# aelmiger/LINE-MOD-Pipeline

Hardware: AMD Instinct MI355X
Metric: detections/sec (higher is better)
Workload: dtype u8

## Files before the change

line-mod-pipeline_amd/csrc/lm_common.h:

```cpp
#pragma once
#include <stdint.h>

typedef uint8_t u8;
typedef uint16_t u16;
typedef uint32_t u32;
typedef uint64_t u64;

#define LM_SCAN_CHUNK 1008
#define LM_SCAN4_CHUNK 1016
#define LM_SCAN_FPAD 8
#define LM_SCANL_LDS_BYTES 163840
#define LM_SCANL_IMAGE_MAX 153600
#define LM_SCANL_TABLE_BYTES 2048
#define LM_SCANL_POS_BITS 15
#define LM_SORT_CAP 4096
#define LM_SORT_CHUNK 1024
#define LM_INLINE_MATCHES 2048
#define LM_DROPPED 0xFFFFFFFFu

struct LmLevelGeom {
    int w, h;
    int T;
    int W, H;
    int spread_only;
    int nibble;
    u32 wh;
    u32 ori_stride;
    u32 plane_ori;
    u32 mod_stride;
    u32 zero_off;
    u32 arena_bytes;
};

struct LmCand {
    u32 ti;
    int x, y;
    float sim;
};

struct LmRefFeat {
    u32 off;
    int16_t x, y;
};

struct LmRefMeta {
    int width, height;
    int nfeat_total;
    u32 start[2];
    u32 count[2];
};

struct LmDevHeader {
    u32 cand_count;
    u32 match_count;
    u32 pad[2];
};

struct LmOutMatch { int x, y; float similarity; int template_id; int class_idx; };

struct LmHeader {
    u32 cand_count;
    u32 match_count;
    u32 out_count;
    u32 sorted_on_device;
};

struct LmHostBlock {
    LmHeader hdr;
    LmOutMatch rec[LM_INLINE_MATCHES];
};
```

line-mod-pipeline_amd/csrc/lm_detector.hip:

```cpp
#include "lm_detector_impl.h"

namespace lmd {

thread_local std::string g_err;
int fail(int code, const std::string& msg) { g_err = msg; return code; }

bool any_lane_busy(const lm_detector* d) {
    for (const lm_detector::Lane& ln : d->lanes) if (ln.busy) return true;
    return false;
}

void free_device_bank(lm_detector* d) {
    hipFree(d->d_item_t); hipFree(d->d_item_chunk); hipFree(d->d_scan_off); hipFree(d->d_scan_P);
    hipFree(d->d_scan_n); hipFree(d->d_t_global); hipFree(d->d_t_class);
    hipFree(d->d_off1); hipFree(d->d_offn); hipFree(d->d_offs3); d->d_off1 = d->d_offn = d->d_offs3 = nullptr;
    hipFree(d->d_offl); hipFree(d->d_offsl); hipFree(d->d_litem); d->d_offl = d->d_offsl = d->d_litem = nullptr;
    for (auto& it : d->items1) { hipFree(it.d_t); hipFree(it.d_chunk); }
    d->items1.clear();
    d->d_item_t = d->d_item_chunk = d->d_scan_off = nullptr;
    d->d_scan_P = d->d_scan_n = d->d_t_global = d->d_t_class = nullptr;
    for (int l = 0; l < LM_MAX_LEVELS; ++l) {
        hipFree(d->d_ref_meta[l]); hipFree(d->d_ref_feat[l]);
        d->d_ref_meta[l] = nullptr; d->d_ref_feat[l] = nullptr;
    }
// ... 357 lines not shown
            for (int l = 0; l < L; ++l) lmk_color_quantize(ln.stream, d->bgr(first, l), d->lw[l], d->lh[l], c.weak_threshold, d->quant(first, l, 0), nullptr, d->cscratch(first, l), fs, n, true);
        grads_done = true;
    }
    for (int l = 0; l < L; ++l) {
        if (l > 0 && !(l == 1 && blur_pyr)) lmk_pyrdown(ln.stream, d->bgr(first, l - 1), d->lw[l - 1], d->lh[l - 1], d->bgr(first, l), fs, n);
        if (!grads_done)
        lmk_color_quantize(ln.stream, d->bgr(first, l), d->lw[l], d->lh[l], c.weak_threshold, d->quant(first, l, 0),
                           nullptr, d->cscratch(first, l), fs, n, l == 0 && blur_pyr);
        if (M == 2 && l == 0)
            lmk_depth_quantize(ln.stream, d->depth(first), d->lw[0], d->lh[0], c.distance_threshold,
                               c.difference_threshold, d->d_normal_lut, normal_lut_onehot(d), d->quant(first, 0, 1),
                               d->dscratch(first), fs, n);
    }
    if (masked) {
        enqueue_mask_rules(d, ln, first, n);
        enqueue_match_masks(d, ln, first, n);
    }
    if (M == 2 && L > 2) enqueue_depth_pyramid(d, ln, first, n);
    for (int l = 0; l < L; ++l)
        for (int m = 0; m < M; ++m) enqueue_lm(d, ln, first, n, l, m, l == L - 1 ? planes : 0u);
}

void fill_raw_thr(int* tab, float threshold) {
    for (int n = 0; n < 128; ++n) tab[n] = static_cast<int>(2 * n + (threshold / 100.f) * (2 * n) + 0.5f);
}

int item_range(lm_detector* d, int class_idx, ItemRange* r) {
    const int nc = (int)d->bank.classes.size();
    if (class_idx >= nc || class_idx < -1) return fail(LM_ERR_INVALID, "class index out of range");
    if (class_idx < 0) { r->lo = 0; r->n = (int)d->hb.item_t.size(); r->t_lo = 0; r->t_hi = (int)d->hb.t_global.size(); }
    else {
        r->lo = d->hb.class_item_lo[class_idx]; r->n = d->hb.class_item_hi[class_idx] - r->lo;
        r->t_lo = d->hb.class_t_lo[class_idx]; r->t_hi = d->hb.class_t_hi[class_idx];
    }
    return LM_OK;
}

int item_ranges(lm_detector* d, std::vector<int>& classes, std::vector<ItemRange>& out) {
    const int nc = (int)d->bank.classes.size();
    out.clear();
    for (int c : classes) if (c < -1 || c >= nc) return fail(LM_ERR_INVALID, "class index out of range");
    std::sort(classes.begin(), classes.end());
    classes.erase(std::unique(classes.begin(), classes.end()), classes.end());
    if (classes.empty() || classes[0] < 0) {
        if (classes.size() > 1) return fail(LM_ERR_INVALID, "class index -1 (all classes) cannot be combined with others");
        classes.assign(1, -1);
        out.push_back(ItemRange{0, (int)d->hb.item_t.size(), 0, (int)d->hb.t_global.size()});
        return LM_OK;
    }
    for (int c : classes) {
        const int lo = d->hb.class_item_lo[c], hi = d->hb.class_item_hi[c];
        if (!out.empty() && out.back().lo + out.back().n == lo && out.back().t_hi == d->hb.class_t_lo[c]) { out.back().n += hi - lo; out.back().t_hi = d->hb.class_t_hi[c]; }
        else out.push_back(ItemRange{lo, hi - lo, d->hb.class_t_lo[c], d->hb.class_t_hi[c]});
    }
    return LM_OK;
}

int ensure_items1(lm_detector* d, int L1, const lm_detector::Items1** out) {
    for (const auto& it : d->items1) if (it.L == L1) { *out = &it; return LM_OK; }
    std::vector<u32> t, c;
    lm_detector::Items1 it;
    it.L = L1;
    lmh::build_items1(d->hb, L1, t, c, it.begin);
    int rc;
    if ((rc = upload_vec(&it.d_t, t))) return rc;
    if ((rc = upload_vec(&it.d_chunk, c))) { hipFree(it.d_t); return rc; }
    d->items1.push_back(std::move(it));
    *out = &d->items1.back();
    return LM_OK;
}

static unsigned slot_layouts(const lm_detector* d, int first, int n) {
    unsigned held = 0;
    for (int i = first; i < first + n; ++i) held |= lmh::layout_bit(d->slots[i].layout);
    return held;
}

static int refuse_scan(lmh::ScanPlan::Kind k) {
    if (k == lmh::ScanPlan::Mixed)
        return fail(LM_ERR_INVALID, "the slots were prepared by calls of different scan forms (some keep only the spread byte of the scanned level): match them apart or upload again");
    return fail(LM_ERR_HIP, "the slots keep only the spread byte of the scanned level and the bit-plane scan could not be set up for them: upload the frames again");
}

int make_scan_args(lm_detector* d, lm_detector::Lane& ln, int first, ItemRange r, int nslots, LmScanArgs* out) {
    const int L = d->cfg.pyramid_levels;
    const LmLevelGeom& g = d->geom[L - 1];
    const unsigned held = slot_layouts(d, first, nslots);
    const bool spread = held == lmh::layout_bit(lmh::Layout::SpreadAndPlanes);
    const int lo = d->hb.lds_ok ? d->hb.lbegin[(size_t)r.t_lo] : 0, nl = d->hb.lds_ok ? d->hb.lbegin[(size_t)r.t_hi] - lo : 0;
    lmh::ScanPlan p = lmh::plan_scan(scan_inputs(d, ln), nslots, held, nl);
    const lm_detector::Items1* it = nullptr;
    if (p.kind == lmh::ScanPlan::Scan1 && ensure_items1(d, p.param, &it) != LM_OK)
        p.kind = spread ? lmh::ScanPlan::NoBitPlaneForm : lmh::ScanPlan::Scan4;
    if (p.kind == lmh::ScanPlan::Mixed || p.kind == lmh::ScanPlan::NoBitPlaneForm) return refuse_scan(p.kind);
    LmScanArgs& a = *out;
    a.L1 = 0; a.G1 = 1; a.L1_rcp16 = 0; a.delta_rcp16 = 0; a.off1 = a.offn = nullptr; a.fpad1 = 0; a.no_exact = 0; a.surv = nullptr; a.surv_cap = 0; a.surv_set = 0; a.exact_spread = 0; a.offs3 = nullptr; a.resp_tab = nullptr;
    a.lm = d->lm(first, L - 1); a.lm_slot_stride = d->frame_stride;
    a.item_t = d->d_item_t; a.item_chunk = d->d_item_chunk;
    a.item_lo = r.lo; a.n_items = r.n;
    a.scan_off = d->d_scan_off; a.scan_P = d->d_scan_P; a.scan_n = d->d_scan_n;
    a.M = d->cfg.num_modalities; a.fpad = d->hb.fpad; a.nibble = g.nibble;
    a.raw_thr_by_n = ln.d_raw_thr;
    a.stat = d->scan_stats ? d->d_scan_stat : nullptr;
    a.W = g.W; a.T = g.T;
    a.hdr = reinterpret_cast<LmDevHeader*>(d->aux(first, d->off_hdr));
    a.cand = reinterpret_cast<LmCand*>(d->aux(first, d->off_cand));
    a.aux_slot_stride = d->aux_stride;
    a.cand_cap = d->max_cand;
    a.dbg = 0; a.lds_form = 0; a.R = 1; a.offl = a.offsl = a.litem = nullptr; a.litem_lo = a.n_litems = 0; a.pb = a.mod_stride = a.planes_off = a.plane_ori = a.tbl_bytes = a.queue_cap = 0;
    if (p.kind != lmh::ScanPlan::Scan4) {
        a.delta_rcp16 = (65536u + (u32)d->miss_delta - 1u) / (u32)d->miss_delta;
        a.fpad1 = d->hb.fpad1; a.exact_spread = spread ? 1 : 0; a.offs3 = d->d_offs3; a.resp_tab = d->d_resp_tab;
    }
    if (p.kind == lmh::ScanPlan::ScanL) {
        a.lds_form = 1; a.R = p.param;
        a.offl = d->d_offl; a.offsl = d->d_offsl; a.litem = d->d_litem; a.litem_lo = lo; a.n_litems = nl;
        a.pb = (u32)g.T * (u32)g.T * g.wh / 8u; a.mod_stride = g.mod_stride; a.planes_off = 8u * g.ori_stride; a.plane_ori = g.plane_ori;
        const u32 img = (u32)a.M * 8u * a.pb;
        a.tbl_bytes = std::max<u32>(LM_SCANL_TABLE_BYTES, (((g.wh + 127u) / 128u) * 16u + 32u + 15u) & ~15u);
        a.queue_cap = std::min<u32>((LM_SCANL_LDS_BYTES - img - a.tbl_bytes - 16u - 512u) / 4u, 1u << 16);
    } else if (p.kind == lmh::ScanPlan::Scan1) {
        const int L1 = p.param;
        a.L1 = L1; a.G1 = 64 / L1;
        a.L1_rcp16 = (65536u + (u32)L1 - 1u) / (u32)L1;
        a.off1 = d->d_off1; a.offn = d->d_offn;
        a.item_t = it->d_t; a.item_chunk = it->d_chunk;
        a.item_lo = it->begin[(size_t)r.t_lo]; a.n_items = it->begin[(size_t)r.t_hi] - a.item_lo;
        unsigned long long*& q = ln.d_surv;
        if (!q) {
            if (hipMalloc(reinterpret_cast<void**>(&q), (16 + (size_t)d->surv_cap) * sizeof(unsigned long long)) != hipSuccess) { q = nullptr; (void)hipGetLastError(); }
            else if (hipMemsetAsync(q, 0, 16 * sizeof(unsigned long long), ln.stream) != hipSuccess) { hipFree(q); q = nullptr; (void)hipGetLastError(); }
            ln.surv_set = 0;
        }
        a.surv = q; a.surv_cap = d->surv_cap;
        a.surv_set = ln.surv_set;
        if (g.wh >= (1u << 20) || nslots > 4096) a.surv = nullptr;
    }
    return LM_OK;
}

void launch_scan(lm_detector::Lane& ln, LmScanArgs& a, int variant, int nslots) {
    lmk_scan(ln.stream, a, variant, nslots);
    if (!a.L1 || !a.surv) return;
    ln.surv_set ^= 1;
    a.surv_set = ln.surv_set;
}

LmRefineArgs make_refine_args(lm_detector* d, int first, int level, float threshold) {
    LmRefineArgs a;
    a.lm = d->lm(first, level); a.lm_slot_stride = d->frame_stride;
    a.g = d->geom[level];
    a.M = d->cfg.num_modalities;
    a.meta = d->d_ref_meta[level]; a.feats = d->d_ref_feat[level];
    a.sim_lut = d->d_sim_lut;
    a.hdr = reinterpret_cast<LmDevHeader*>(d->aux(first, d->off_hdr));
    a.cand = reinterpret_cast<LmCand*>(d->aux(first, d->off_cand));
    a.keys = reinterpret_cast<u64*>(d->aux(first, d->off_keys));
    a.aux_slot_stride = d->aux_stride;
    a.cand_cap = d->max_cand; a.match_cap = d->max_match;
    a.threshold = threshold;
    a.t_global = d->d_t_global; a.t_class = d->d_t_class;
    a.plan = nullptr; a.plan_cap = 0;
    a.stat = d->d_refine_stat;
    return a;
}

LmSortArgs make_sort_args(lm_detector* d, int first) {
    LmSortArgs a;
    a.hdr = reinterpret_cast<LmDevHeader*>(d->aux(first, d->off_hdr));
    a.keys = reinterpret_cast<u64*>(d->aux(first, d->off_keys));
    a.out = reinterpret_cast<LmOutMatch*>(d->aux(first, d->off_out));
    a.split = d->sort_split_mode == 1 || (d->sort_split_mode == 2 && d->sort_long_score > 0);
    a.aux_slot_stride = d->aux_stride;
    a.host = d->host_block(first);
    a.host_slot_stride = d->host_stride;
    a.cand_cap = d->max_cand; a.match_cap = d->max_match;
    return a;
}

int enqueue_threshold(lm_detector::Lane& ln, float threshold) {
    if (!(threshold >= 0.0f)) return fail(LM_ERR_INVALID, "threshold must be >= 0");
    if (ln.raw_thr_for != threshold) {
        HIP_TRY(hipStreamSynchronize(ln.stream));
        fill_raw_thr(ln.h_raw_thr, threshold);
        HIP_TRY(hipMemcpyAsync(ln.d_raw_thr, ln.h_raw_thr, 128 * sizeof(int), hipMemcpyHostToDevice, ln.stream));
        ln.raw_thr_for = threshold;
    }
    return LM_OK;
}

int enqueue_match_stages(lm_detector* d, lm_detector::Lane& ln, int first, int n, float threshold, const std::vector<ItemRange>& ranges, bool timed) {
    const int L = d->cfg.pyramid_levels;
    if (lmh::layouts_mixed(slot_layouts(d, first, n))) return refuse_scan(lmh::ScanPlan::Mixed);
    if (timed) HIP_TRY(hipEventRecord(ln.ev[1], ln.stream));
    for (const ItemRange& r : ranges)
        if (r.n > 0) {
            LmScanArgs sa;
            if (int rc = make_scan_args(d, ln, first, r, n, &sa)) return rc;
            launch_scan(ln, sa, d->scan_variant, n);
            d->cnt_scan_launches += 1; d->cnt_scan1_launches += (sa.L1 || sa.lds_form) ? 1 : 0; d->last_scan1_lanes = scan_form_code(sa);
        }
    if (timed) HIP_TRY(hipEventRecord(ln.ev[2], ln.stream));
    if (L == 1) {
        lmk_emit_unrefined(ln.stream, make_refine_args(d, first, 0, threshold), n);
    } else {
        u32* plan = nullptr;
        const int plan_cap = n / 8 + 8;
        if ((n % 8) == 0 && n <= 1016 && plan_cap <= d->plan_stride_cap && ln.plan) {
            plan = ln.plan;
            lmk_refine_plan(ln.stream, make_refine_args(d, first, L - 2, threshold), n, plan, plan_cap);
        }
        for (int l = L - 2; l >= 0; --l) {
            LmRefineArgs ra = make_refine_args(d, first, l, threshold);
            ra.plan = plan; ra.plan_cap = plan_cap;
            lmk_refine(ln.stream, ra, l == 0, n);
            d->cnt_refine_launches += 1;
        }
    }
    if (timed) HIP_TRY(hipEventRecord(ln.ev[3], ln.stream));
    lmk_sort_unique(ln.stream, make_sort_args(d, first), n);
    d->cnt_sort_launches += 1;
    if (timed) HIP_TRY(hipEventRecord(ln.ev[4], ln.stream));
    HIP_TRY(hipGetLastError());
    return LM_OK;
}

int enqueue_upload_wait(lm_detector* d, lm_detector::Lane& ln, int first, int n) {
    int rc;
    unsigned long long seqs[LM_NCOPY];
    if ((rc = wait_uploads(d, ln.stream, first, n, seqs))) return rc;
    for (int k = 0; k < LM_NCOPY; ++k) if (seqs[k] > ln.waited_seq[k]) ln.waited_seq[k] = seqs[k];
    return LM_OK;
}

int enqueue_match(lm_detector* d, lm_detector::Lane& ln, int first, int n, float threshold, std::vector<int>& classes, bool timed,
                  bool prepared) {
    std::vector<ItemRange> ranges;
    int rc;
    if ((rc = item_ranges(d, classes, ranges))) return rc;
    if ((rc = enqueue_threshold(ln, threshold))) return rc;
    if ((rc = enqueue_upload_wait(d, ln, first, n))) return rc;
    if (timed) HIP_TRY(hipEventRecord(ln.ev[0], ln.stream));
    if (!prepared) {
        enqueue_preprocess(d, ln, first, n);
        d->cnt_preprocess_frames += n;
        for (int i = 0; i < n; ++i) d->slots[first + i].prepared = true;
    }
    return enqueue_match_stages(d, ln, first, n, threshold, ranges, timed);
}
int enqueue_match(lm_detector* d, lm_detector::Lane& ln, int first, int n, float threshold, int class_idx, bool timed) {
    std::vector<int> classes(1, class_idx);
    return enqueue_match(d, ln, first, n, threshold, classes, timed);
}

inline bool key_less(const u64* a, const u64* b) { return a[0] < b[0] || (a[0] == b[0] && a[1] < b[1]); }

int collect_slot(lm_detector* d, int slot, lm_match_t* out, size_t cap, size_t* n_out) {
    const LmHostBlock* hb = d->host_block(slot);
    const LmHeader h = hb->hdr;
    if (h.cand_count > d->max_cand)
        return fail(LM_ERR_OVERFLOW, "scan produced " + std::to_string(h.cand_count) + " candidates, capacity " +
                                         std::to_string(d->max_cand) + " (raise lm_config.max_candidates)");
    if (h.match_count > d->max_match)
        return fail(LM_ERR_OVERFLOW, "refinement produced " + std::to_string(h.match_count) + " matches, capacity " +
                                         std::to_string(d->max_match) + " (raise lm_config.max_matches)");
    note_sort_length(d, h.match_count);
    size_t n = 0;
    if (h.sorted_on_device) {
        n = h.out_count;
        size_t ncopy = std::min(n, cap);
        size_t inl = std::min<size_t>(ncopy, LM_INLINE_MATCHES);
        if (out && inl) std::memcpy(out, hb->rec, inl * sizeof(lm_match_t));
        if (out && ncopy > inl)
            HIP_TRY(hipMemcpy(out + inl, reinterpret_cast<lm_match_t*>(d->aux(slot, d->off_out)) + inl,
                              (ncopy - inl) * sizeof(lm_match_t), hipMemcpyDeviceToHost));
    } else {
        std::vector<u64> keys((size_t)h.match_count * 2);
        if (h.match_count)
            HIP_TRY(hipMemcpy(keys.data(), d->aux(slot, d->off_keys), keys.size() * sizeof(u64), hipMemcpyDeviceToHost));
        std::vector<u32> idx(h.match_count);
        for (u32 i = 0; i < h.match_count; ++i) idx[i] = i;
        std::sort(idx.begin(), idx.end(), [&](u32 a, u32 b) { return key_less(&keys[2 * (size_t)a], &keys[2 * (size_t)b]); });
        const u64* prev = nullptr;
        for (u32 i : idx) {
            const u64* k = &keys[2 * (size_t)i];
            if (prev && prev[1] == k[1] && (prev[0] >> 32) == (k[0] >> 32)) { prev = k; continue; }
            prev = k;
            if (out && n < cap) {
                lm_match_t m;
                u32 sb = ~(u32)(k[0] >> 32);
                std::memcpy(&m.similarity, &sb, 4);
                m.template_id = (int)(u32)k[0];
                m.class_idx = (int)(k[1] >> 48);
                m.y = (int)((k[1] >> 24) & 0xFFFFFFu) - 0x800000;
                m.x = (int)(k[1] & 0xFFFFFFu) - 0x800000;
                out[n] = m;
            }
            ++n;
        }
    }
    if (n_out) *n_out = n;
    if (n > cap && out) return fail(LM_ERR_OVERFLOW, "output buffer too small for " + std::to_string(n) + " matches");
    return LM_OK;
}

int ready_for_compute(lm_detector* d) {
    int rc;
    if (!d) return fail(LM_ERR_INVALID, "null detector");
    if ((rc = ensure_device(d))) return rc;
    if ((rc = ensure_luts(d))) return rc;
    return LM_OK;
}

int ensure_scratch(lm_detector* d, size_t bytes) {
    if (bytes <= d->scratch_bytes) return LM_OK;
    HIP_TRY(hipDeviceSynchronize());
    hipFree(d->d_scratch);
    d->d_scratch = nullptr; d->scratch_bytes = 0;
    HIP_TRY(hipMalloc(&d->d_scratch, bytes));
    d->scratch_bytes = bytes;
    return LM_OK;
}

int ensure_lane(lm_detector* d, int l) {
    lm_detector::Lane& ln = d->lanes[l];
    if (ln.created) return LM_OK;
    if (!ln.stream) HIP_TRY(hipStreamCreateWithFlags(&ln.stream, hipStreamNonBlocking));
    for (auto& e : ln.ev) HIP_TRY(hipEventCreate(&e));
    HIP_TRY(hipMalloc(reinterpret_cast<void**>(&ln.d_raw_thr), 128 * sizeof(int)));
    HIP_TRY(hipHostMalloc(reinterpret_cast<void**>(&ln.h_raw_thr), 128 * sizeof(int), hipHostMallocDefault));
    ln.raw_thr_for = -1.0f;
    ln.created = true;
    return LM_OK;
}

void account_profile(lm_detector* d, const lm_detector::Lane& ln, int n, const std::vector<int>& classes, bool gathered) {
    for (int k = 0; k < 4; ++k) {
        float ms = 0;
        if (hipEventElapsedTime(&ms, ln.ev[k], ln.ev[k + 1]) == hipSuccess) d->prof_us[k] += (double)ms * 1000.0;
    }
    if (gathered) {
        float ms = 0;
        if (hipEventElapsedTime(&ms, ln.ev[4], ln.ev[5]) == hipSuccess) { d->prof_exch_us += (double)ms * 1000.0; d->prof_exch_launches += 1; }
    }
    double b = 0;
    for (int c : classes) {
        if (c < 0) for (double v : d->hb.class_alg_bytes) b += v;
        else if (c < (int)d->hb.class_alg_bytes.size()) b += d->hb.class_alg_bytes[c];
    }
    d->prof_scan_bytes += b * n;
    d->prof_launches += 1;
    d->prof_frames += n;
}

int wait_stream(lm_detector* d, lm_detector::Lane& ln) {
    if (d->cfg.flags & LM_FLAG_BLOCKING_SYNC) {
        hipEvent_t& ev = ln.blocking_ev;
        if (!ev) HIP_TRY(hipEventCreateWithFlags(&ev, hipEventBlockingSync | hipEventDisableTiming));
        HIP_TRY(hipEventRecord(ev, ln.stream));
        HIP_TRY(hipEventSynchronize(ev));
    } else {
        HIP_TRY(hipStreamSynchronize(ln.stream));
    }
    for (int k = 0; k < LM_NCOPY; ++k) if (ln.waited_seq[k] > d->up_seq_done[k]) d->up_seq_done[k] = ln.waited_seq[k];
    return LM_OK;
}

int wait_lane_done(lm_detector* d, lm_detector::Lane& ln) {
    HIP_TRY(hipEventSynchronize(ln.ev_done));
    for (int k = 0; k < LM_NCOPY; ++k) if (ln.waited_seq[k] > d->up_seq_done[k]) d->up_seq_done[k] = ln.waited_seq[k];
    return LM_OK;
}

int run_match(lm_detector* d, lm_detector::Lane& ln, int first, int n, float threshold, std::vector<int> classes, bool prepared = false) {
    if (any_lane_busy(d)) return fail(LM_ERR_INVALID, "a lane has a match in flight: call lm_match_end first");
    for (int i = 0; i < n; ++i) {
        if (!d->slots[first + i].has_frame) return fail(LM_ERR_INVALID, "no frame uploaded to slot " + std::to_string(first + i));
        if (prepared && !d->slots[first + i].prepared)
            return fail(LM_ERR_INVALID, "slot " + std::to_string(first + i) + " holds no current a3-a10 results: run lm_prepare_slot or a match on it first");
    }
    int rc;
    if ((rc = enqueue_match(d, ln, first, n, threshold, classes, d->profiling, prepared))) return rc;
    if ((rc = wait_stream(d, ln))) return rc;
    if (d->profiling) account_profile(d, ln, n, classes);
    for (int i = 0; i < n; ++i) d->slots[first + i].matched = true;
    return LM_OK;
}
int run_match(lm_detector* d, lm_detector::Lane& ln, int first, int n, float threshold, int class_idx) {
    return run_match(d, ln, first, n, threshold, std::vector<int>(1, class_idx));
}

}

extern "C" {

const char* lm_last_error(void) { return g_err.c_str(); }
const char* lm_version(void) { return "linemod_hip 0.9 (gfx950; the 0.8 ABI plus the mask rules, lm_set_mask_rule; 0.8 = the 0.7 ABI plus lm_icp_verify*; 0.7 = the 0.6 ABI plus lm_pose_error_*; 0.6 = the 0.5 ABI plus template generation; 0.5 = the 0.4 ABI plus lm_icp_*)"; }

void lm_default_config(lm_config* c, int color_only, int width, int height) {
    std::memset(c, 0, sizeof(*c));
    c->width = width; c->height = height;
    c->num_modalities = color_only ? 1 : 2;
    c->pyramid_levels = 2;
    c->T[0] = color_only ? 2 : 5;
    c->T[1] = 8;
    c->weak_threshold = 10.0f; c->num_features = 63; c->strong_threshold = 55.0f;
    c->distance_threshold = 2000; c->difference_threshold = 50; c->depth_num_features = 63; c->extract_threshold = 2;
    c->device = 0; c->shard_rank = 0; c->shard_size = 1;
    c->max_candidates = 0; c->max_matches = 0; c->frame_slots = 0;
}

int lm_create(const lm_config* cfg, lm_detector** out) {
    if (!cfg || !out) return fail(LM_ERR_INVALID, "null argument");
    *out = nullptr;
    lm_config c = *cfg;
    if (c.num_modalities < 1 || c.num_modalities > 2) return fail(LM_ERR_INVALID, "num_modalities must be 1 or 2");
    if (c.pyramid_levels < 1 || c.pyramid_levels > LM_MAX_LEVELS) return fail(LM_ERR_INVALID, "pyramid_levels out of range");
    if (c.width <= 0 || c.height <= 0) return fail(LM_ERR_INVALID, "bad frame size");
    if (c.shard_size < 1 || c.shard_rank < 0 || c.shard_rank >= c.shard_size) return fail(LM_ERR_INVALID, "bad shard rank/size");
    if (c.max_candidates <= 0) c.max_candidates = 1 << 18;
    if (c.max_matches <= 0) c.max_matches = 1 << 18;
    if (c.frame_slots <= 0) c.frame_slots = 8;
    if (c.frame_slots > 1024) return fail(LM_ERR_INVALID, "frame_slots out of range");
    {
        std::string why;
        if (!lmh::check_modality_params(c, why)) return fail(LM_ERR_INVALID, why);
    }
    lm_detector* d = new lm_detector();
    d->cfg = c;
    d->max_cand = (u32)c.max_candidates;
    d->max_match = (u32)c.max_matches;
    int w = c.width, h = c.height;
    for (int l = 0; l < c.pyramid_levels; ++l) {
        if (l > 0) { w /= 2; h /= 2; }
        int T = c.T[l];
        if (T <= 0 || w <= 0 || h <= 0 || w % T || h % T || ((long long)w * h) % 16) {
            delete d;
            return fail(LM_ERR_INVALID, "frame size violates cols%T==0, rows%T==0, (rows*cols)%16==0 at level " + std::to_string(l));
        }
        d->lw[l] = w; d->lh[l] = h;
        LmLevelGeom& g = d->geom[l];
        g.w = w; g.h = h; g.T = T; g.W = w / T; g.H = h / T;
        g.wh = (u32)g.W * (u32)g.H;
        size_t pad = align_up((size_t)g.wh + 16 * (size_t)g.W + 2 * LM_SCAN_CHUNK + 64, 256);
        g.spread_only = (l + 1 < c.pyramid_levels) ? 1 : 0;
        g.nibble = (!g.spread_only && !(c.flags & LM_FLAG_BYTE_RESPONSES) && lmk_nibble_supported(w, h, T)) ? 1 : 0;
        size_t ori = align_up(((size_t)T * T * g.wh) >> g.nibble, 256) + pad;
        size_t plane = g.nibble ? align_up(((size_t)T * T * g.wh + 7) / 8 + ((size_t)g.wh + 64 * 128) / 8 + 64, 256) : 0;
        if (g.nibble && (size_t)c.num_modalities * (8 * ori + 8 * plane) + pad > 0x1FFFFFFFull) plane = 0;
        size_t mod = g.spread_only ? ori : 8 * ori + 8 * plane;
        size_t arena = (size_t)c.num_modalities * mod + pad;
        if (arena > (g.spread_only ? 0x1FFFFFFFull : g.nibble ? 0x7FFFFFFFull : 0xFFFFFFFFull)) { delete d; return fail(LM_ERR_INVALID, "frame too large for the arena offset encoding"); }
        g.ori_stride = (u32)ori;
        g.plane_ori = (u32)plane;
        g.mod_stride = (u32)mod;
        g.zero_off = (u32)((size_t)c.num_modalities * g.mod_stride);
        g.arena_bytes = (u32)arena;
    }
    lmh::default_similarity_lut(d->sim_lut);
    lmh::default_normal_lut(d->normal_lut);
    if (const char* ev = getenv("LM_SCANL_R")) d->scanl_R = std::max(1, atoi(ev));
    *out = d;
    return LM_OK;
}


void lm_destroy(lm_detector* d) {
    if (!d) return;
    if (d->dev_ready) {
        hipSetDevice(d->cfg.device);
        hipDeviceSynchronize();
        if (d->d_refine_stat) {
            unsigned long long h[8] = {};
            if (hipMemcpy(h, d->d_refine_stat, sizeof(h), hipMemcpyDeviceToHost) == hipSuccess)
                fprintf(stderr, "LM_REFINE_STAT: refined alone %llu, in pairs %llu | pair candidates pruned %llu (both of a pair: %llu pairs) | single candidates pruned %llu | dropped by the final test %llu\n",
                        h[0], h[1], h[2], h[3], h[4], h[5]);
            hipFree(d->d_refine_stat);
        }
        for (Slot& s : d->slots) {
            if (s.h_bgr) hipHostFree(s.h_bgr);
            if (s.h_depth) hipHostFree(s.h_depth);
            if (s.ev_up) hipEventDestroy(s.ev_up);
            if (s.ev_bgr) hipEventDestroy(s.ev_bgr);
            if (s.h_match_mask) hipHostFree(s.h_match_mask);
            hipFree(s.d_match_mask);
            hipFree(s.d_rule_mask);
        }
        for (auto& cs : d->copy_stream) if (cs) hipStreamDestroy(cs);
        free_icp(d);
        free_gen(d);
        free_eval(d);
        hipFree(d->frame_arena); hipFree(d->aux_arena); hipHostFree(d->host_blocks);
        hipFree(d->d_plan);
        for (lm_detector::Lane& ln : d->lanes) {
            hipFree(ln.d_surv); hipFree(ln.d_raw_thr);
            if (ln.h_raw_thr) hipHostFree(ln.h_raw_thr);
            for (hipEvent_t ev : ln.ev) if (ev) hipEventDestroy(ev);
            for (hipEvent_t ev : {ln.ev_done, ln.blocking_ev, ln.mask_done}) if (ev) hipEventDestroy(ev);
            if (ln.stream) hipStreamDestroy(ln.stream);
            delete ln.comm; ln.comm = nullptr;
        }
        free_device_bank(d);
        free_gather(d);
        hipFree(d->d_scan_stat);
        hipFree(d->d_hull_class_base); hipFree(d->d_hull_off); hipFree(d->d_hull_xy); hipFree(d->d_hsv_div);
        if (d->cc_stream) hipStreamDestroy(d->cc_stream);
        hipFree(d->cc_dev); if (d->cc_host) hipHostFree(d->cc_host);
        hipFree(d->dc_dev); if (d->dc_host) hipHostFree(d->dc_host);
        if (d->cc_done) hipEventDestroy(d->cc_done);
        if (d->dc_done) hipEventDestroy(d->dc_done);
        hipFree(d->d_resp_tab); hipFree(d->d_sim_lut); hipFree(d->d_normal_lut); hipFree(d->d_scratch);
    }
    delete d;
}

int lm_set_similarity_lut(lm_detector* d, const uint8_t lut[256]) {
    if (d && any_lane_busy(d)) return fail(LM_ERR_INVALID, "a lane has a match in flight: call lm_match_end first");
    if (!d || !lut) return fail(LM_ERR_INVALID, "null argument");
    for (int i = 0; i < 256; ++i) if (lut[i] > 4) return fail(LM_ERR_INVALID, "similarity LUT entries must be <= 4 (63*4 must fit a byte)");
    for (int o = 0; o < 8; ++o) if (lut[32 * o] || lut[32 * o + 16]) return fail(LM_ERR_INVALID, "similarity LUT must map an empty nibble to 0");
    std::memcpy(d->sim_lut, lut, 256); d->luts_dirty = true;
    for (Slot& sl : d->slots) sl.prepared = false;
    return LM_OK;
}
int lm_set_normal_lut(lm_detector* d, const uint8_t lut[8000]) {
    if (d && any_lane_busy(d)) return fail(LM_ERR_INVALID, "a lane has a match in flight: call lm_match_end first");
    if (!d || !lut) return fail(LM_ERR_INVALID, "null argument");
    std::memcpy(d->normal_lut, lut, 8000); d->luts_dirty = true; d->lut_onehot = -1; d->normal_lut_substitute = false;
    for (Slot& sl : d->slots) sl.prepared = false;
    return LM_OK;
}
int lm_get_similarity_lut(const lm_detector* d, uint8_t lut[256]) { if (!d || !lut) return fail(LM_ERR_INVALID, "null argument"); std::memcpy(lut, d->sim_lut, 256); return LM_OK; }
int lm_normal_lut_is_substitute(const lm_detector* d) { return (d && d->normal_lut_substitute) ? 1 : 0; }
int lm_get_normal_lut(const lm_detector* d, uint8_t lut[8000]) { if (!d || !lut) return fail(LM_ERR_INVALID, "null argument"); std::memcpy(lut, d->normal_lut, 8000); return LM_OK; }

int lm_num_classes(const lm_detector* d) { return d ? (int)d->bank.classes.size() : -1; }
int lm_num_templates(const lm_detector* d) {
    if (!d) return -1;
    int n = 0;
    for (const auto& c : d->bank.classes) n += (int)c.pyramids.size();
    return n;
}
int lm_class_num_templates(const lm_detector* d, int ci) {
    if (!d || ci < 0 || ci >= (int)d->bank.classes.size()) return -1;
    return (int)d->bank.classes[ci].pyramids.size();
}
const char* lm_class_id(const lm_detector* d, int ci) {
    if (!d || ci < 0 || ci >= (int)d->bank.classes.size()) return nullptr;
    return d->bank.classes[ci].id.c_str();
}
int lm_find_class(const lm_detector* d, const char* id) { return (d && id) ? d->bank.find(id) : -1; }
int lm_get_T(const lm_detector* d, int level) { return (d && level >= 0 && level < d->cfg.pyramid_levels) ? d->cfg.T[level] : -1; }
int lm_num_modalities(const lm_detector* d) { return d ? d->cfg.num_modalities : -1; }
int lm_pyramid_levels(const lm_detector* d) { return d ? d->cfg.pyramid_levels : -1; }

int lm_add_class(lm_detector* d, const char* class_id, int n_templates, const lm_template_desc* descs,
                 const lm_feature* features, int* class_idx_out) {
    if (d && any_lane_busy(d)) return fail(LM_ERR_INVALID, "a lane has a match in flight: call lm_match_end first");
    if (!d || !class_id || n_templates < 0 || (n_templates && (!descs || !features))) return fail(LM_ERR_INVALID, "null argument");
    std::string err;
    int ci = d->bank.add_class(class_id, n_templates, descs, features, d->cfg.pyramid_levels, d->cfg.num_modalities, err);
    if (ci < 0) return fail(LM_ERR_INVALID, err);
    if (class_idx_out) *class_idx_out = ci;
    d->bank_dirty = true; d->hulls_dirty = true;
    return LM_OK;
}

int lm_add_template(lm_detector* d, const char* class_id, const uint8_t* bgr, size_t bgr_stride, const uint16_t* depth,
                    size_t depth_stride, const uint8_t* mask, size_t mask_stride, int* template_id_out, lm_rect* bbox_out) {
    if (d && any_lane_busy(d)) return fail(LM_ERR_INVALID, "a lane has a match in flight: call lm_match_end first");
    if (template_id_out) *template_id_out = -1;
    int rc;
    if ((rc = ready_for_compute(d))) return rc;
    if (!class_id) return fail(LM_ERR_INVALID, "null class id");
    const lm_config& c = d->cfg;
    const int M = c.num_modalities, L = c.pyramid_levels;
    hipStream_t st = d->lanes[0].stream;
    if ((rc = upload_frame(d, 0, bgr, bgr_stride, depth, depth_stride, inline_on(st)))) return rc;
    d->slots[0].has_frame = false;
    d->slots[0].prepared = false;
    size_t mag_off[LM_MAX_LEVELS], total = 0;
    for (int l = 0; l < L; ++l) { mag_off[l] = total; total += align_up((size_t)d->lw[l] * d->lh[l] * sizeof(float), 256); }
    if ((rc = ensure_scratch(d, total))) return rc;
    u8* scratch = static_cast<u8*>(d->d_scratch);
    for (int l = 0; l < L; ++l) {
        if (l > 0) lmk_pyrdown(st, d->bgr(0, l - 1), d->lw[l - 1], d->lh[l - 1], d->bgr(0, l), 0, 1);
        lmk_color_quantize(st, d->bgr(0, l), d->lw[l], d->lh[l], c.weak_threshold, d->quant(0, l, 0),
                           reinterpret_cast<float*>(scratch + mag_off[l]), d->cscratch(0, l), 0, 1);
    }
    if (M == 2) {
        lmk_depth_quantize(st, d->depth(0), d->lw[0], d->lh[0], c.distance_threshold, c.difference_threshold,
                           d->d_normal_lut, normal_lut_onehot(d), d->quant(0, 0, 1), d->dscratch(0), 0, 1);
        enqueue_depth_pyramid(d, d->lanes[0], 0, 1);
    }
    std::vector<lmh::ExtractLevel> lv(L);
    for (int l = 0; l < L; ++l) {
        size_t px = (size_t)d->lw[l] * d->lh[l];
        lv[l].w = d->lw[l]; lv[l].h = d->lh[l];
        lv[l].color_q.resize(px); lv[l].color_mag.resize(px);
        HIP_TRY(hipMemcpyAsync(lv[l].color_q.data(), d->quant(0, l, 0), px, hipMemcpyDeviceToHost, st));
        HIP_TRY(hipMemcpyAsync(lv[l].color_mag.data(), scratch + mag_off[l], px * sizeof(float), hipMemcpyDeviceToHost, st));
        if (M == 2) {
            lv[l].depth_q.resize(px);
// ... 292 lines not shown
```

line-mod-pipeline_amd/csrc/lm_detector_debug.hip:

```cpp
#include "lm_detector_impl.h"

extern "C" {

int lm_stage_color_quantize(lm_detector* d, const uint8_t* bgr, int w, int h, float weak_threshold, uint8_t* quantized,
                            float* magnitude) {
    int rc;
    if ((rc = ready_for_compute(d))) return rc;
    if (!bgr || !quantized || w <= 0 || h <= 0) return fail(LM_ERR_INVALID, "bad argument");
    size_t px = (size_t)w * h;
    size_t o_q = align_up(px * 3 + 256, 256), o_m = o_q + align_up(px, 256), o_s = o_m + align_up(px * 4, 256);
    if ((rc = ensure_scratch(d, o_s + lmk_color_scratch_bytes(w, h)))) return rc;
    u8* base = static_cast<u8*>(d->d_scratch);
    hipStream_t st = d->lanes[0].stream;
    HIP_TRY(hipMemcpyAsync(base, bgr, px * 3, hipMemcpyHostToDevice, st));
    lmk_color_quantize(st, base, w, h, weak_threshold, base + o_q, magnitude ? reinterpret_cast<float*>(base + o_m) : nullptr,
                       base + o_s, 0, 1);
    HIP_TRY(hipMemcpyAsync(quantized, base + o_q, px, hipMemcpyDeviceToHost, st));
    if (magnitude) HIP_TRY(hipMemcpyAsync(magnitude, base + o_m, px * 4, hipMemcpyDeviceToHost, st));
    HIP_TRY(hipStreamSynchronize(st));
    HIP_TRY(hipGetLastError());
    return LM_OK;
}

int lm_stage_pyrdown(lm_detector* d, const uint8_t* bgr, int w, int h, uint8_t* out) {
    int rc;
    if ((rc = ready_for_compute(d))) return rc;
    if (!bgr || !out || w < 2 || h < 2) return fail(LM_ERR_INVALID, "bad argument");
    size_t px = (size_t)w * h, opx = (size_t)(w / 2) * (h / 2);
    size_t o_o = align_up(px * 3, 256);
    if ((rc = ensure_scratch(d, o_o + opx * 3))) return rc;
    u8* base = static_cast<u8*>(d->d_scratch);
    hipStream_t st = d->lanes[0].stream;
    HIP_TRY(hipMemcpyAsync(base, bgr, px * 3, hipMemcpyHostToDevice, st));
    lmk_pyrdown(st, base, w, h, base + o_o, 0, 1);
    HIP_TRY(hipMemcpyAsync(out, base + o_o, opx * 3, hipMemcpyDeviceToHost, st));
    HIP_TRY(hipStreamSynchronize(st));
    HIP_TRY(hipGetLastError());
    return LM_OK;
}

int lm_stage_depth_quantize(lm_detector* d, const uint16_t* depth, int w, int h, uint8_t* quantized) {
    int rc;
    if ((rc = ready_for_compute(d))) return rc;
    if (!depth || !quantized || w <= 0 || h <= 0) return fail(LM_ERR_INVALID, "bad argument");
    size_t px = (size_t)w * h;
    size_t o_q = align_up(px * 2, 256), o_s = o_q + align_up(px, 256);
    if ((rc = ensure_scratch(d, o_s + px))) return rc;
    u8* base = static_cast<u8*>(d->d_scratch);
    hipStream_t st = d->lanes[0].stream;
    HIP_TRY(hipMemcpyAsync(base, depth, px * 2, hipMemcpyHostToDevice, st));
    lmk_depth_quantize(st, reinterpret_cast<u16*>(base), w, h, d->cfg.distance_threshold, d->cfg.difference_threshold,
                       d->d_normal_lut, normal_lut_onehot(d), base + o_q, base + o_s, 0, 1);
    HIP_TRY(hipMemcpyAsync(quantized, base + o_q, px, hipMemcpyDeviceToHost, st));
    HIP_TRY(hipStreamSynchronize(st));
    HIP_TRY(hipGetLastError());
    return LM_OK;
}

int lm_stage_linear_memories(lm_detector* d, const uint8_t* quantized, int w, int h, int T, uint8_t* out) {
    int rc;
    if ((rc = ready_for_compute(d))) return rc;
    if (!quantized || !out || w <= 0 || h <= 0 || T <= 0 || w % T || h % T) return fail(LM_ERR_INVALID, "bad argument");
    size_t px = (size_t)w * h;
    size_t o_l = align_up(px, 256);
    if ((rc = ensure_scratch(d, o_l + 8 * px))) return rc;
    u8* base = static_cast<u8*>(d->d_scratch);
    hipStream_t st = d->lanes[0].stream;
    HIP_TRY(hipMemcpyAsync(base, quantized, px, hipMemcpyHostToDevice, st));
    lmk_linear_memories(st, base, w, 0, 0, w, h, T, d->d_resp_tab, base + o_l, (u32)px, 0, 0, 1);
    HIP_TRY(hipMemcpyAsync(out, base + o_l, 8 * px, hipMemcpyDeviceToHost, st));
    HIP_TRY(hipStreamSynchronize(st));
    HIP_TRY(hipGetLastError());
    return LM_OK;
}

int lm_stage_mask_rule(lm_detector* d, const uint8_t* bgr, const uint16_t* depth, int w, int h, const lm_mask_rule* rule, uint8_t* mask_out) {
    int rc;
    if ((rc = ready_for_compute(d))) return rc;
    if (!rule || !mask_out) return fail(LM_ERR_INVALID, "null argument");
    if (w != d->cfg.width || h != d->cfg.height) return fail(LM_ERR_INVALID, "lm_stage_mask_rule takes images of the detector's size");
    LmRuleArgs a{};
    if ((rc = check_mask_rule(d, rule, &a.rule[0]))) return rc;
    if ((a.rule[0].use_hsv && !bgr) || (a.rule[0].use_depth && !depth)) return fail(LM_ERR_INVALID, "the rule gates on an image that is missing");
    if (a.rule[0].use_hsv && (rc = ensure_hsv_div(d))) return rc;
    const size_t px = (size_t)w * h, pitch = d->match_mask_pitch;
    const size_t o_d = align_up(px * 3, 256), o_m = o_d + align_up(px * 2, 256);
    if ((rc = ensure_scratch(d, o_m + pitch * h))) return rc;
    u8* base = static_cast<u8*>(d->d_scratch);
    hipStream_t st = d->lanes[0].stream;
    if (a.rule[0].use_hsv) HIP_TRY(hipMemcpyAsync(base, bgr, px * 3, hipMemcpyHostToDevice, st));
    if (a.rule[0].use_depth) HIP_TRY(hipMemcpyAsync(base + o_d, depth, px * 2, hipMemcpyHostToDevice, st));
    a.bgr = base; a.depth = reinterpret_cast<const u16*>(base + o_d); a.slot_stride = 0; a.divtab = d->d_hsv_div;
    a.w = w; a.h = h; a.mask_pitch = (u32)pitch;
    a.n = 1; a.slot[0] = 0; a.kind[0] = 0; a.plane[0] = base + o_m;
    lmk_mask_rule(st, a);
    HIP_TRY(hipMemcpy2DAsync(mask_out, (size_t)w, base + o_m, pitch, (size_t)w, (size_t)h, hipMemcpyDeviceToHost, st));
    HIP_TRY(hipStreamSynchronize(st));
    HIP_TRY(hipGetLastError());
    return LM_OK;
}

int lm_prepare_slot(lm_detector* d, int slot) {
    int rc;
    if ((rc = ready_for_compute(d))) return rc;
    if ((rc = check_slots(d, slot, 1))) return rc;
    if (!d->slots[slot].has_frame) return fail(LM_ERR_INVALID, "no frame uploaded to slot");
    lm_detector::Lane& ln = d->lanes[0];
    if ((rc = enqueue_upload_wait(d, ln, slot, 1))) return rc;
    enqueue_preprocess(d, ln, slot, 1);
    d->cnt_preprocess_frames += 1;
    if ((rc = wait_stream(d, ln))) return rc;
    HIP_TRY(hipGetLastError());
    d->slots[slot].prepared = true;
    return LM_OK;
}

int lm_debug_read(lm_detector* d, int slot, int what, int level, int modality, uint8_t* out, size_t cap, size_t* size_out) {
    int rc;
    if ((rc = ready_for_compute(d))) return rc;
    if ((rc = check_slots(d, slot, 1))) return rc;
    if (level < 0 || level >= d->cfg.pyramid_levels || modality < 0 || modality >= d->cfg.num_modalities)
        return fail(LM_ERR_INVALID, "level/modality out of range");
    lm_detector::Lane& ln = d->lanes[0];
    HIP_TRY(hipStreamSynchronize(ln.stream));
    const LmLevelGeom& g = d->geom[level];
    if (what == 0) {
        size_t n = (size_t)g.w * g.h;
        if (size_out) *size_out = n;
        if (modality == 1 && level > 0) {
            enqueue_depth_pyramid(d, ln, slot, 1);
            HIP_TRY(hipStreamSynchronize(ln.stream));
        }
        if (out) HIP_TRY(hipMemcpy(out, d->quant(slot, level, modality), std::min(n, cap), hipMemcpyDeviceToHost));
        return LM_OK;
    }
    if (what == 1) {
        size_t blk = (size_t)g.T * g.T * g.wh;
        if (!g.spread_only) return fail(LM_ERR_INVALID, "the lowest level keeps response memories, not the spread memory");
        if (size_out) *size_out = blk;
        if (out) {
            if (cap < blk) return fail(LM_ERR_INVALID, "buffer too small");
            HIP_TRY(hipMemcpy(out, d->lm(slot, level) + (size_t)modality * g.mod_stride, blk, hipMemcpyDeviceToHost));
        }
        return LM_OK;
    }
    if (what == 2) {
        size_t blk = (size_t)g.T * g.T * g.wh;
        size_t n = 8 * blk;
        if (size_out) *size_out = n;
        if (out) {
            if (cap < n) return fail(LM_ERR_INVALID, "buffer too small");
            if (g.spread_only || (level == d->cfg.pyramid_levels - 1 && d->slots[slot].layout == lmh::Layout::SpreadAndPlanes)) {
                std::vector<u8> sp(blk);
                HIP_TRY(hipMemcpy(sp.data(), d->lm(slot, level) + (size_t)modality * g.mod_stride, blk, hipMemcpyDeviceToHost));
                for (int o = 0; o < 8; ++o)
                    for (size_t i = 0; i < blk; ++i)
                        out[o * blk + i] = std::max(d->sim_lut[32 * o + (sp[i] & 15)], d->sim_lut[32 * o + 16 + (sp[i] >> 4)]);
            } else if (g.nibble) {
                std::vector<u8> pk(blk / 2);
                for (int o = 0; o < 8; ++o) {
                    HIP_TRY(hipMemcpy(pk.data(), d->lm(slot, level) + (size_t)modality * g.mod_stride + (size_t)o * g.ori_stride,
                                      blk / 2, hipMemcpyDeviceToHost));
                    for (size_t i = 0; i < blk / 2; ++i) { out[o * blk + 2 * i] = pk[i] & 15; out[o * blk + 2 * i + 1] = pk[i] >> 4; }
                }
            } else {
                for (int o = 0; o < 8; ++o)
                    HIP_TRY(hipMemcpy(out + o * blk, d->lm(slot, level) + (size_t)modality * g.mod_stride + (size_t)o * g.ori_stride, blk,
                                      hipMemcpyDeviceToHost));
            }
        }
        return LM_OK;
    }
    return fail(LM_ERR_INVALID, "unknown buffer id");
}

int lm_stage_scan(lm_detector* d, int slot, float threshold, int class_idx, int32_t* out, size_t cap_records, size_t* n_out) {
    int rc;
    if ((rc = ready_for_compute(d))) return rc;
    if ((rc = check_slots(d, slot, 1))) return rc;
    if ((rc = ensure_bank(d))) return rc;
    ItemRange r;
    if ((rc = item_range(d, class_idx, &r))) return rc;
    lm_detector::Lane& ln = d->lanes[0];
    if ((rc = enqueue_threshold(ln, threshold))) return rc;
    {
        LmScanArgs sa;
        if ((rc = make_scan_args(d, ln, slot, r, 1, &sa))) return rc;
        launch_scan(ln, sa, d->scan_variant, 1);
        d->last_scan1_lanes = scan_form_code(sa);
    }
    LmDevHeader h;
    HIP_TRY(hipMemcpyAsync(&h, d->aux(slot, d->off_hdr), sizeof(h), hipMemcpyDeviceToHost, ln.stream));
    HIP_TRY(hipStreamSynchronize(ln.stream));
    HIP_TRY(hipGetLastError());
    HIP_TRY(hipMemsetAsync(d->aux(slot, d->off_hdr), 0, sizeof(LmDevHeader), ln.stream));
    HIP_TRY(hipStreamSynchronize(ln.stream));
    if (h.cand_count > d->max_cand) return fail(LM_ERR_OVERFLOW, "candidate buffer overflow");
    std::vector<LmCand> cand(h.cand_count);
    if (h.cand_count) HIP_TRY(hipMemcpy(cand.data(), d->aux(slot, d->off_cand), cand.size() * sizeof(LmCand), hipMemcpyDeviceToHost));
    struct Rec { int32_t tid, cls, x, y; };
    std::vector<Rec> recs(cand.size());
    for (size_t i = 0; i < cand.size(); ++i)
        recs[i] = Rec{d->hb.t_global[cand[i].ti], d->hb.t_class[cand[i].ti], cand[i].x, cand[i].y};
    std::sort(recs.begin(), recs.end(), [](const Rec& a, const Rec& b) {
        if (a.cls != b.cls) return a.cls < b.cls;
        if (a.tid != b.tid) return a.tid < b.tid;
        if (a.y != b.y) return a.y < b.y;
        return a.x < b.x;
    });
    if (n_out) *n_out = recs.size();
    if (out) std::memcpy(out, recs.data(), std::min(recs.size(), cap_records) * sizeof(Rec));
    return LM_OK;
}

int lm_time_scan(lm_detector* d, int slot, float threshold, int class_idx, int iters, int variant, double* avg_us_out,
                 double* algorithmic_bytes_out) {
    int rc;
    if ((rc = ready_for_compute(d))) return rc;
    if ((rc = check_slots(d, slot, 1))) return rc;
    if ((rc = ensure_bank(d))) return rc;
    if (iters <= 0) return fail(LM_ERR_INVALID, "iters must be positive");
    ItemRange r;
    if ((rc = item_range(d, class_idx, &r))) return rc;
    lm_detector::Lane& ln = d->lanes[0];
    if ((rc = enqueue_threshold(ln, threshold))) return rc;
    LmScanArgs a;
    if ((rc = make_scan_args(d, ln, slot, r, 1, &a))) return rc;
    a.cand_cap = 0;
    for (int i = 0; i < 3; ++i) launch_scan(ln, a, variant, 1);
    HIP_TRY(hipEventRecord(ln.ev[0], ln.stream));
    for (int i = 0; i < iters; ++i) launch_scan(ln, a, variant, 1);
    HIP_TRY(hipEventRecord(ln.ev[1], ln.stream));
    HIP_TRY(hipMemsetAsync(d->aux(slot, d->off_hdr), 0, sizeof(LmDevHeader), ln.stream));
    HIP_TRY(hipStreamSynchronize(ln.stream));
    HIP_TRY(hipGetLastError());
    float ms = 0;
    HIP_TRY(hipEventElapsedTime(&ms, ln.ev[0], ln.ev[1]));
    if (avg_us_out) *avg_us_out = (double)ms * 1000.0 / iters;
    if (algorithmic_bytes_out) {
        double b = 0;
        if (class_idx < 0) for (double v : d->hb.class_alg_bytes) b += v;
        else b = d->hb.class_alg_bytes[class_idx];
        *algorithmic_bytes_out = b;
    }
    return LM_OK;
}

int lm_time_scan_batch(lm_detector* d, int first_slot, int n_slots, float threshold, int class_idx, int iters, int variant,
                       double* avg_us_out) {
    int rc;
    if ((rc = ready_for_compute(d))) return rc;
    if ((rc = check_slots(d, first_slot, n_slots))) return rc;
    if ((rc = ensure_bank(d))) return rc;
    if (iters <= 0 || n_slots <= 0) return fail(LM_ERR_INVALID, "iters and n_slots must be positive");
    if (any_lane_busy(d)) return fail(LM_ERR_INVALID, "a lane has a match in flight: call lm_match_end first");
    for (int i = 0; i < n_slots; ++i)
        if (!d->slots[first_slot + i].prepared) return fail(LM_ERR_INVALID, "slot " + std::to_string(first_slot + i) + " is not prepared");
    ItemRange r;
    if ((rc = item_range(d, class_idx, &r))) return rc;
    lm_detector::Lane& ln = d->lanes[0];
    if ((rc = enqueue_threshold(ln, threshold))) return rc;
    LmScanArgs a;
    if ((rc = make_scan_args(d, ln, first_slot, r, n_slots, &a))) return rc;
    a.cand_cap = 0;
    for (int i = 0; i < 2; ++i) launch_scan(ln, a, variant, n_slots);
    HIP_TRY(hipEventRecord(ln.ev[0], ln.stream));
    for (int i = 0; i < iters; ++i) launch_scan(ln, a, variant, n_slots);
    HIP_TRY(hipEventRecord(ln.ev[1], ln.stream));
    for (int i = 0; i < n_slots; ++i) HIP_TRY(hipMemsetAsync(d->aux(first_slot + i, d->off_hdr), 0, sizeof(LmDevHeader), ln.stream));
    HIP_TRY(hipStreamSynchronize(ln.stream));
    HIP_TRY(hipGetLastError());
    float ms = 0;
    HIP_TRY(hipEventElapsedTime(&ms, ln.ev[0], ln.ev[1]));
    if (avg_us_out) *avg_us_out = (double)ms * 1000.0 / iters;
    return LM_OK;
}

int lm_selftest_float_tail(lm_detector* d, uint64_t out[8]) {
    int rc;
    if (!out) return fail(LM_ERR_INVALID, "null argument");
    if ((rc = ready_for_compute(d))) return rc;
    if (any_lane_busy(d)) return fail(LM_ERR_INVALID, "a lane has a match in flight: call lm_match_end first");
    unsigned long long* dev = nullptr;
    HIP_TRY(hipMalloc(reinterpret_cast<void**>(&dev), 8 * sizeof(unsigned long long)));
    lm_detector::Lane& ln = d->lanes[0];
    hipError_t e = hipMemsetAsync(dev, 0, 8 * sizeof(unsigned long long), ln.stream);
    unsigned long long host[8] = {0, 0, 0, 0, 0, 0, 0, 0};
    if (e == hipSuccess) { lmk_selftest_float_tail(ln.stream, dev); e = hipMemcpyAsync(host, dev, sizeof(host), hipMemcpyDeviceToHost, ln.stream); }
    if (e == hipSuccess) e = hipStreamSynchronize(ln.stream);
    if (e == hipSuccess) e = hipGetLastError();
    (void)hipFree(dev);
    if (e != hipSuccess) return fail(LM_ERR_HIP, hipGetErrorString(e));
    for (int k = 0; k < 8; ++k) out[k] = host[k];
    return LM_OK;
}

int lm_time_stages(lm_detector* d, int slot, float threshold, int class_idx, int iters, double out_us[4]) {
    int rc;
    if ((rc = ready_for_compute(d))) return rc;
    if ((rc = check_slots(d, slot, 1))) return rc;
    if ((rc = ensure_bank(d))) return rc;
    if (iters <= 0 || !out_us) return fail(LM_ERR_INVALID, "bad argument");
    if (!d->slots[slot].has_frame) return fail(LM_ERR_INVALID, "no frame uploaded to slot");
    double acc[4] = {0, 0, 0, 0};
    lm_detector::Lane& ln = d->lanes[0];
    for (int it = 0; it < iters; ++it) {
        if ((rc = enqueue_match(d, ln, slot, 1, threshold, class_idx, true))) return rc;
// ... 138 lines not shown
```

line-mod-pipeline_amd/csrc/lm_dev_memories.h:

```cpp
#pragma once
#include "lm_dev.h"

namespace {

#define LMK_MAX_LOADS 8
template <int SRC_SHIFT, bool SPREAD_ONLY>
__global__ __launch_bounds__(256) void k_linear_memories(const u8* __restrict__ q0, int qpitch, int w, int h, int T,
                                                          int seg, const u64* __restrict__ resp_tab,
                                                          u8* __restrict__ lm0, u32 ori_stride, size_t q_slot_stride,
                                                          size_t lm_slot_stride) {
    extern __shared__ __attribute__((aligned(16))) u8 smem[];
    const u8* q = slot_ptr(q0, q_slot_stride);
    u8* lm = slot_ptr(lm0, lm_slot_stride);
    const int W = w / T;
    const u32 wh = (u32)W * (u32)(h / T);
    const int rows = 2 * T - 1;
    const int pitch = (seg * T + T + 3) & ~3;
    u64* tab = reinterpret_cast<u64*>(smem);
    u8* qs = smem + 2048;
    u8* ho = qs + rows * pitch;
    const int tid = threadIdx.x;
    const int band = blockIdx.y;
    const int col0 = blockIdx.x * seg;
    const int ncols = (W - col0) < seg ? (W - col0) : seg;
    const int px0 = col0 * T, npx = ncols * T;
    const int y0 = band * T;
    const int lw = npx + T - 1;

    tab[tid] = resp_tab[tid];
    {
        const int total = rows * lw;
        u8 v[LMK_MAX_LOADS];
#pragma unroll
        for (int k = 0; k < LMK_MAX_LOADS; ++k) {
            int i = tid + k * 256;
            int yy = i / lw, xx = i - yy * lw;
            int gy = y0 + yy, gx = px0 + xx;
            u8 val = 0;
            if (i < total && gy < h && gx < w)
                val = SRC_SHIFT ? q[(size_t)(2 * gy) * qpitch + 2 * gx] : q[(size_t)gy * qpitch + gx];
            v[k] = val;
        }
#pragma unroll
        for (int k = 0; k < LMK_MAX_LOADS; ++k) {
            int i = tid + k * 256;
            if (i < total) { int yy = i / lw; qs[yy * pitch + (i - yy * lw)] = v[k]; }
        }
    }
    __syncthreads();
    for (int i = tid; i < rows * npx; i += 256) {
        int yy = i / npx, xx = i - yy * npx;
        const u8* p = qs + yy * pitch + xx;
        u8 v = 0;
        for (int c = 0; c < T; ++c) v |= p[c];
        ho[yy * pitch + xx] = v;
    }
    __syncthreads();
    if ((W & 3) == 0 && (seg & 3) == 0) {
        const int C4 = ncols >> 2;
        const int units = T * T * C4;
        for (int u = tid; u < units; u += 256) {
            int k4 = u % C4, g = u / C4;
            int j = g / T, c0 = g - j * T;
            u8 sv[4];
#pragma unroll
            for (int i = 0; i < 4; ++i) {
                int x = (4 * k4 + i) * T + c0;
                const u8* p = ho + j * pitch + x;
                u8 acc = 0;
                for (int r = 0; r < T; ++r) acc |= p[r * pitch];
                sv[i] = acc;
            }
            u8* dst = lm + (size_t)g * wh + (size_t)band * W + col0 + 4 * k4;
            if (SPREAD_ONLY) {
                *reinterpret_cast<u32*>(dst) = (u32)sv[0] | ((u32)sv[1] << 8) | ((u32)sv[2] << 16) | ((u32)sv[3] << 24);
            } else {
                u64 e0 = tab[sv[0]], e1 = tab[sv[1]], e2 = tab[sv[2]], e3 = tab[sv[3]];
#pragma unroll
                for (int o = 0; o < 8; ++o) {
                    u32 v = (u32)((e0 >> (8 * o)) & 0xFF) | ((u32)((e1 >> (8 * o)) & 0xFF) << 8) |
                            ((u32)((e2 >> (8 * o)) & 0xFF) << 16) | ((u32)((e3 >> (8 * o)) & 0xFF) << 24);
                    *reinterpret_cast<u32*>(dst + (size_t)o * ori_stride) = v;
                }
            }
        }
    } else {
        const int units = T * T * ncols;
        for (int u = tid; u < units; u += 256) {
            int k = u % ncols, g = u / ncols;
            int j = g / T, c0 = g - j * T;
            const u8* p = ho + j * pitch + k * T + c0;
            u8 sv = 0;
            for (int r = 0; r < T; ++r) sv |= p[r * pitch];
            u8* dst = lm + (size_t)g * wh + (size_t)band * W + col0 + k;
            if (SPREAD_ONLY) {
                dst[0] = sv;
            } else {
                u64 e = tab[sv];
#pragma unroll
                for (int o = 0; o < 8; ++o) dst[(size_t)o * ori_stride] = (u8)(e >> (8 * o));
            }
        }
    }
}

__device__ __host__ __forceinline__ void bit_transpose8(u32& x, u32& y) {
    u32 t;
    t = (y ^ (y >> 7)) & 0x00AA00AAu; y = y ^ t ^ (t << 7);
    t = (x ^ (x >> 7)) & 0x00AA00AAu; x = x ^ t ^ (t << 7);
    t = (y ^ (y >> 14)) & 0x0000CCCCu; y = y ^ t ^ (t << 14);
    t = (x ^ (x >> 14)) & 0x0000CCCCu; x = x ^ t ^ (t << 14);
    t = (y & 0xF0F0F0F0u) | ((x >> 4) & 0x0F0F0F0Fu);
    x = ((y << 4) & 0xF0F0F0F0u) | (x & 0x0F0F0F0Fu);
    y = t;
}

template <int T, int SEG, int SRC_SHIFT, int MODE>
__device__ __forceinline__ void d_lm_fast(const u32 vblock, const u8* __restrict__ q0, int qpitch, int w, int h,
                                                  const u64* __restrict__ resp_tab, u8* __restrict__ lm0,
                                                  u32 ori_stride, size_t q_slot_stride, size_t lm_slot_stride,
                                                  int nseg, int nslots, u32 plane_ori = 0) {
    constexpr int ROWS = 2 * T - 1;
    constexpr int TW = SEG * T;
    constexpr int NDW = (TW + T - 1 + 3) / 4;
    constexpr int PD = NDW + 2;
    constexpr int NLOAD = (ROWS * PD + 255) / 256;
    constexpr bool SPREAD_ONLY = MODE == 1;
    __shared__ u64 tab[SPREAD_ONLY ? 1 : 256];
    __shared__ u8 tabu[MODE == 2 ? 256 : 1];
    __shared__ u32 qs[ROWS][PD];
    __shared__ u32 ho[ROWS][PD];
    __shared__ u32 sp[T][PD];
    u32 slot, tile;
    xcd_slot_tile_b(vblock, (u32)(nseg * (h / T)), (u32)nslots, slot, tile);
    const u8* q = slot_ptr_s(q0, q_slot_stride, slot);
    u8* lm = slot_ptr_s(lm0, lm_slot_stride, slot);
    const int tid = threadIdx.x;
    const int W = w / T;
    const u32 wh = (u32)W * (u32)(h / T);
    const int band = (int)(tile / (u32)nseg);
    const int col0 = (int)(tile - (u32)band * (u32)nseg) * SEG;
    const int ncols = (W - col0) < SEG ? (W - col0) : SEG;
    const int px0 = col0 * T, y0 = band * T;

    if (!SPREAD_ONLY) tab[tid] = resp_tab[tid];
    if (MODE == 2 && plane_ori) tabu[tid] = reinterpret_cast<const u8*>(resp_tab + 256)[tid];
    {
        u32 v[NLOAD];
#pragma unroll
        for (int k = 0; k < NLOAD; ++k) {
            const int i = tid + k * 256;
            const int r = i / PD, c = i - r * PD;
            const int gy = y0 + r, gx = px0 + 4 * c;
            u32 val = 0;
            if (i < ROWS * PD && c < NDW && gy < h && gx < w) {
                if (SRC_SHIFT) {
                    const u32* sp2 = reinterpret_cast<const u32*>(q + (size_t)(2 * gy) * qpitch + 2 * gx);
                    val = __builtin_amdgcn_perm(sp2[1], sp2[0], 0x06040200u);
                } else {
                    val = *reinterpret_cast<const u32*>(q + (size_t)gy * qpitch + gx);
                }
            }
            v[k] = val;
        }
#pragma unroll
        for (int k = 0; k < NLOAD; ++k) {
            const int i = tid + k * 256;
            if (i < ROWS * PD) { const int r = i / PD; qs[r][i - r * PD] = v[k]; }
        }
    }
    __syncthreads();
    for (int i = tid; i < ROWS * NDW; i += 256) {
        const int r = i / NDW, c = i - r * NDW;
        const u32 d0 = qs[r][c], d1 = qs[r][c + 1], d2 = qs[r][c + 2];
        u32 hor = d0;
#pragma unroll
        for (int k = 1; k < T; ++k) {
            if (k < 4) hor |= __builtin_amdgcn_alignbyte(d1, d0, (u32)k);
            else if (k == 4) hor |= d1;
            else hor |= __builtin_amdgcn_alignbyte(d2, d1, (u32)(k - 4));
        }
        ho[r][c] = hor;
    }
    __syncthreads();
    for (int i = tid; i < T * NDW; i += 256) {
        const int j = i / NDW, c = i - j * NDW;
        u32 v = 0;
#pragma unroll
        for (int r = 0; r < T; ++r) v |= ho[j + r][c];
        sp[j][c] = v;
    }
    __syncthreads();
    if (MODE == 2) {
        constexpr int UW = (T == 8 && SEG == 80) ? 16 : 8;
        constexpr int NH = UW / 8;
        constexpr int CU = SEG / UW;
        const bool spread_low = (plane_ori >> 31) != 0;
        plane_ori &= 0x7FFFFFFFu;
        for (int u = tid; u < T * T * CU; u += 256) {
            const int ku = u % CU, g = u / CU;
            const int j = g / T, c0 = g - j * T;
            if (UW * ku >= ncols) continue;
            const u8* row = reinterpret_cast<const u8*>(&sp[j][0]);
            u32 nd[NH][8], pb[NH][8];
            u32 sb[NH][2];
#pragma unroll
            for (int h = 0; h < NH; ++h) {
                const int k8 = NH * ku + h;
                if (spread_low) {
                    sb[h][0] = sb[h][1] = 0;
#pragma unroll
                    for (int i = 0; i < 4; ++i) {
                        sb[h][0] |= (u32)row[(8 * k8 + i) * T + c0] << (8 * i);
                        sb[h][1] |= (u32)row[(8 * k8 + 4 + i) * T + c0] << (8 * i);
                    }
                }
#pragma unroll
                for (int o = 0; o < 8; ++o) nd[h][o] = 0;
                if (!spread_low) {
                    u64 e[4];
#pragma unroll
                    for (int i = 0; i < 4; ++i)
                        e[i] = tab[row[(8 * k8 + 2 * i) * T + c0]] | (tab[row[(8 * k8 + 2 * i + 1) * T + c0]] << 4);
                    const u32 a0 = (u32)e[0], a1 = (u32)e[1], a2 = (u32)e[2], a3 = (u32)e[3];
                    const u32 b0 = (u32)(e[0] >> 32), b1 = (u32)(e[1] >> 32), b2 = (u32)(e[2] >> 32), b3 = (u32)(e[3] >> 32);
#pragma unroll
                    for (int o = 0; o < 4; ++o) {
                        const u32 sel = (u32)o | ((u32)(o + 4) << 8);
                        nd[h][o] = (__builtin_amdgcn_perm(a1, a0, sel) & 0xFFFFu) | (__builtin_amdgcn_perm(a3, a2, sel) << 16);
                        nd[h][o + 4] = (__builtin_amdgcn_perm(b1, b0, sel) & 0xFFFFu) | (__builtin_amdgcn_perm(b3, b2, sel) << 16);
                    }
                }
                if (plane_ori) {
                    u32 x = 0, y = 0;
#pragma unroll
                    for (int i = 0; i < 4; ++i) {
                        x |= (u32)tabu[row[(8 * k8 + i) * T + c0]] << (8 * i);
                        y |= (u32)tabu[row[(8 * k8 + 4 + i) * T + c0]] << (8 * i);
                    }
                    bit_transpose8(x, y);
#pragma unroll
                    for (int o = 0; o < 4; ++o) { pb[h][o] = (x >> (8 * o)) & 0xFFu; pb[h][o + 4] = (y >> (8 * o)) & 0xFFu; }
                }
            }
            const size_t pos = (size_t)g * wh + (size_t)band * W + col0 + UW * ku;
            u8* dst = lm + (pos >> 1);
            u8* pl = lm + 8 * (size_t)ori_stride + (pos >> 3);
            if (spread_low) {
                if (NH == 2) *reinterpret_cast<u32x4*>(lm + pos) = u32x4{sb[0][0], sb[0][1], sb[NH - 1][0], sb[NH - 1][1]};
                else *reinterpret_cast<u32x2*>(lm + pos) = u32x2{sb[0][0], sb[0][1]};
            }
#pragma unroll
            for (int o = 0; o < 8; ++o) {
                if (!spread_low) {
                    if (NH == 2) *reinterpret_cast<u32x2*>(dst + (size_t)o * ori_stride) = u32x2{nd[0][o], nd[NH - 1][o]};
                    else *reinterpret_cast<u32*>(dst + (size_t)o * ori_stride) = nd[0][o];
                }
                if (plane_ori) {
                    if (NH == 2) *reinterpret_cast<unsigned short*>(pl + (size_t)o * plane_ori) = (unsigned short)(pb[0][o] | (pb[NH - 1][o] << 8));
                    else pl[(size_t)o * plane_ori] = (u8)pb[0][o];
                }
            }
        }
        return;
    }
    constexpr int C4 = SEG / 4;
    for (int u = tid; u < T * T * C4; u += 256) {
        const int k4 = u % C4, g = u / C4;
        const int j = g / T, c0 = g - j * T;
        if (4 * k4 >= ncols) continue;
        const u8* row = reinterpret_cast<const u8*>(&sp[j][0]);
        const u32 s0 = row[(4 * k4 + 0) * T + c0], s1 = row[(4 * k4 + 1) * T + c0];
        const u32 s2 = row[(4 * k4 + 2) * T + c0], s3 = row[(4 * k4 + 3) * T + c0];
        u8* dst = lm + (size_t)g * wh + (size_t)band * W + col0 + 4 * k4;
        if (SPREAD_ONLY) {
            *reinterpret_cast<u32*>(dst) = s0 | (s1 << 8) | (s2 << 16) | (s3 << 24);
        } else {
            const u64 e0 = tab[s0], e1 = tab[s1], e2 = tab[s2], e3 = tab[s3];
            const u32 a0 = (u32)e0, a1 = (u32)e1, a2 = (u32)e2, a3 = (u32)e3;
            const u32 b0 = (u32)(e0 >> 32), b1 = (u32)(e1 >> 32), b2 = (u32)(e2 >> 32), b3 = (u32)(e3 >> 32);
#pragma unroll
            for (int o = 0; o < 4; ++o) {
                const u32 sel = (u32)o | ((u32)(o + 4) << 8);
                u32 lo = __builtin_amdgcn_perm(a1, a0, sel) & 0xFFFFu;
                u32 hi = __builtin_amdgcn_perm(a3, a2, sel) << 16;
                *reinterpret_cast<u32*>(dst + (size_t)o * ori_stride) = lo | hi;
                u32 lo2 = __builtin_amdgcn_perm(b1, b0, sel) & 0xFFFFu;
                u32 hi2 = __builtin_amdgcn_perm(b3, b2, sel) << 16;
                *reinterpret_cast<u32*>(dst + (size_t)(o + 4) * ori_stride) = lo2 | hi2;
            }
        }
    }
}
template <int T, int SEG, int SRC_SHIFT, int MODE>
__global__ __launch_bounds__(256) void k_lm_fast(const u8* __restrict__ q0, int qpitch, int w, int h,
                                                  const u64* __restrict__ resp_tab, u8* __restrict__ lm0,
                                                  u32 ori_stride, size_t q_slot_stride, size_t lm_slot_stride,
                                                  int nseg, int nslots, u32 plane_ori) {
    d_lm_fast<T, SEG, SRC_SHIFT, MODE>(blockIdx.x, q0, qpitch, w, h, resp_tab, lm0, ori_stride, q_slot_stride, lm_slot_stride, nseg, nslots, plane_ori);
}

__device__ __forceinline__ void d_lm_spread2(const u32 vblock, const u8* __restrict__ q0, int qpitch, int w, int h, u8* __restrict__ lm0,
                                                     size_t q_slot_stride, size_t lm_slot_stride, int gblocks, int nslots) {
    u32 slot, tile;
    xcd_slot_tile_b(vblock, (u32)gblocks, (u32)nslots, slot, tile);
    const u8* q = slot_ptr_s(q0, q_slot_stride, slot);
    u8* lm = slot_ptr_s(lm0, lm_slot_stride, slot);
    const int ng = w >> 5, W = w >> 1;
    const u32 wh = (u32)W * (u32)(h >> 1);
    const int gid = (int)(tile * 256u) + (int)threadIdx.x;
    const int yp = gid / ng, g = gid - yp * ng;
    const int y = 2 * yp;
    if (y >= h) return;
    u32 R[3][9];
#pragma unroll
    for (int j = 0; j < 3; ++j) {
        const bool in = y + j < h;
        const u8* row = q + (size_t)min(y + j, h - 1) * qpitch + 32 * g;
        const u32x4 a = ld16(row), b = ld16(row + 16);
        const u32 nx = g + 1 < ng ? *reinterpret_cast<const u32*>(row + 32) : 0u;
        R[j][0] = in ? a[0] : 0u; R[j][1] = in ? a[1] : 0u; R[j][2] = in ? a[2] : 0u; R[j][3] = in ? a[3] : 0u;
        R[j][4] = in ? b[0] : 0u; R[j][5] = in ? b[1] : 0u; R[j][6] = in ? b[2] : 0u; R[j][7] = in ? b[3] : 0u;
        R[j][8] = in ? nx : 0u;
    }
#pragma unroll
    for (int r = 0; r < 2; ++r) {
        u32 sp[8];
#pragma unroll
        for (int d = 0; d < 8; ++d) {
            const u32 v0 = R[r][d] | R[r + 1][d], v1 = R[r][d + 1] | R[r + 1][d + 1];
            sp[d] = v0 | __builtin_amdgcn_alignbyte(v1, v0, 1u);
        }
        u32 ev[4], od[4];
#pragma unroll
        for (int k = 0; k < 4; ++k) {
            ev[k] = __builtin_amdgcn_perm(sp[2 * k + 1], sp[2 * k], 0x06040200u);
            od[k] = __builtin_amdgcn_perm(sp[2 * k + 1], sp[2 * k], 0x07050301u);
        }
        if (y + r < h) {
            u8* base = lm + (size_t)(2 * r) * wh + (size_t)yp * W + 16 * g;
            st16(base, u32x4{ev[0], ev[1], ev[2], ev[3]});
            st16(base + wh, u32x4{od[0], od[1], od[2], od[3]});
        }
    }
}
__global__ __launch_bounds__(256) void k_lm_spread2(const u8* __restrict__ q0, int qpitch, int w, int h, u8* __restrict__ lm0,
                                                     size_t q_slot_stride, size_t lm_slot_stride, int gblocks, int nslots) {
    d_lm_spread2(blockIdx.x, q0, qpitch, w, h, lm0, q_slot_stride, lm_slot_stride, gblocks, nslots);
}

__device__ __forceinline__ u32 gather4_stride5(const u32 (&V)[11], int b0) {
    const int a0 = b0, a1 = b0 + 5, a2 = b0 + 10, a3 = b0 + 15;
    const u32 lo = __builtin_amdgcn_perm(V[a1 >> 2], V[a0 >> 2], (u32)(a0 & 3) | ((u32)(4 + (a1 & 3)) << 8) | 0x0c0c0000u);
    const u32 hi = __builtin_amdgcn_perm(V[a3 >> 2], V[a2 >> 2], (u32)(a2 & 3) | ((u32)(4 + (a3 & 3)) << 8) | 0x0c0c0000u);
    return __builtin_amdgcn_perm(hi, lo, 0x05040100u);
}
__device__ __forceinline__ void d_lm_spread5(const u32 vblock, const u8* __restrict__ q0, int qpitch, int w, int h, u8* __restrict__ lm0,
                                             size_t q_slot_stride, size_t lm_slot_stride, int gblocks, int nslots) {
    u32 slot, tile;
    xcd_slot_tile_b(vblock, (u32)gblocks, (u32)nslots, slot, tile);
    const u8* q = slot_ptr_s(q0, q_slot_stride, slot);
    u8* lm = slot_ptr_s(lm0, lm_slot_stride, slot);
    const int W = w / 5, HB = h / 5, ng = W >> 3;
    const u32 wh = (u32)W * (u32)HB;
    const int gid = (int)(tile * 256u) + (int)threadIdx.x;
    const int band = gid / ng, g = gid - band * ng;
    if (band >= HB) return;
    const int x0 = 40 * g, y0 = 5 * band;
    const bool full = x0 + 48 <= w;
    u32 Hr[9][11];
#pragma unroll
    for (int r = 0; r < 9; ++r) {
        u32 R[12];
#pragma unroll
        for (int d = 0; d < 12; ++d) R[d] = 0;
        if (y0 + r < h) {
            const u8* row = q + (size_t)(y0 + r) * qpitch + x0;
            const u32x4 a = ld16a4(row), b = ld16a4(row + 16);
            R[0] = a[0]; R[1] = a[1]; R[2] = a[2]; R[3] = a[3]; R[4] = b[0]; R[5] = b[1]; R[6] = b[2]; R[7] = b[3];
            if (full) { const u32x4 c = ld16a4(row + 32); R[8] = c[0]; R[9] = c[1]; R[10] = c[2]; R[11] = c[3]; }
            else { const u32x2 c = ld8a4(row + 32); R[8] = c[0]; R[9] = c[1]; }
        }
#pragma unroll
        for (int d = 0; d < 11; ++d)
            Hr[r][d] = R[d] | __builtin_amdgcn_alignbyte(R[d + 1], R[d], 1u) | __builtin_amdgcn_alignbyte(R[d + 1], R[d], 2u) |
                       __builtin_amdgcn_alignbyte(R[d + 1], R[d], 3u) | R[d + 1];
    }
#pragma unroll
    for (int j = 0; j < 5; ++j) {
        u32 V[11];
#pragma unroll
        for (int d = 0; d < 11; ++d) V[d] = Hr[j][d] | Hr[j + 1][d] | Hr[j + 2][d] | Hr[j + 3][d] | Hr[j + 4][d];
        u8* dst = lm + (size_t)(j * 5) * wh + (size_t)band * W + 8 * g;
#pragma unroll
        for (int c0 = 0; c0 < 5; ++c0)
            *reinterpret_cast<u32x2*>(dst + (size_t)c0 * wh) = u32x2{gather4_stride5(V, c0), gather4_stride5(V, c0 + 20)};
    }
}
__global__ __launch_bounds__(256) void k_lm_spread5(const u8* __restrict__ q0, int qpitch, int w, int h, u8* __restrict__ lm0,
                                                     size_t q_slot_stride, size_t lm_slot_stride, int gblocks, int nslots) {
    d_lm_spread5(blockIdx.x, q0, qpitch, w, h, lm0, q_slot_stride, lm_slot_stride, gblocks, nslots);
}


}
```

line-mod-pipeline_amd/csrc/lm_host.cpp:

```cpp
#include "lm_host.h"
#if defined(__x86_64__)
#include <immintrin.h>
#endif

#include <algorithm>
#include <cmath>
#include <cstdio>
#include <cstdlib>
#include <cstring>

namespace lmh {

int Bank::find(const std::string& id) const {
    for (size_t i = 0; i < classes.size(); ++i)
        if (classes[i].id == id) return (int)i;
    return -1;
}

int Bank::add_pyramid(const std::string& id, TemplatePyramid&& tp) {
    int ci = find(id);
    if (ci < 0) { classes.push_back(ClassEntry{id, {}}); ci = (int)classes.size() - 1; }
    classes[ci].pyramids.push_back(std::move(tp));
    return (int)classes[ci].pyramids.size() - 1;
}
// ... 67 lines not shown
            tp[k].features.assign(features + fo, features + fo + ds.num_features);
            fo += ds.num_features;
        }
        classes[ci].pyramids.push_back(std::move(tp));
    }
    return ci;
}

void schedule_lds_lists(DeviceBankHost& out);
bool build_device_bank(const Bank& bank, const lm_config& cfg, const LmLevelGeom* geom, DeviceBankHost& out,
                       int scan_list_order, std::string& err) {
    const int M = cfg.num_modalities, L = cfg.pyramid_levels;
    out = DeviceBankHost();
    const LmLevelGeom& gl = geom[L - 1];
    int maxf = 1;
    for (const ClassEntry& c : bank.classes)
        for (const TemplatePyramid& tp : c.pyramids)
            for (int m = 0; m < M; ++m) maxf = std::max(maxf, (int)tp[(size_t)(L - 1) * M + m].features.size());
    const int fq = gl.nibble ? 1 : LM_SCAN_FPAD;
    const u32 osc = gl.nibble ? 2u : 1u;
    out.fpad = (maxf + fq - 1) / fq * fq;
    const int nc = (int)bank.classes.size();
    out.class_item_lo.assign(nc, 0); out.class_item_hi.assign(nc, 0);
    out.class_t_lo.assign(nc, 0); out.class_t_hi.assign(nc, 0);
    out.class_alg_bytes.assign(nc, 0.0);
    out.class_load_bytes.assign(nc, 0.0);
    const bool planes = gl.nibble && gl.plane_ori != 0;
    if (planes) out.fpad1 = (std::min(M * maxf, 2 * LM_MAX_FEATURES) + 7) / 8 * 8;
    const u32 ttwh = (u32)gl.T * (u32)gl.T * gl.wh, pb = ttwh / 8u;
    out.lds_ok = lds_image_fits(gl, M);
    auto plane_bit_off = [&](u32 noff) {
        const u32 base = noff / 2u, m = base / gl.mod_stride, label = (base - m * gl.mod_stride) / gl.ori_stride;
        const u32 rest = noff - 2u * (m * gl.mod_stride + label * gl.ori_stride);
        return 8u * (m * gl.mod_stride + 8u * gl.ori_stride + label * gl.plane_ori) + rest;
    };
    for (int ci = 0; ci < nc; ++ci) {
        const ClassEntry& c = bank.classes[ci];
        int lo, hi;
        shard_range((int)c.pyramids.size(), cfg.shard_rank, cfg.shard_size, &lo, &hi);
        out.class_t_lo[ci] = (int)out.t_global.size();
        out.class_item_lo[ci] = (int)out.item_t.size();
        if (out.lds_ok) while (out.litem.size() % 64u) out.litem.push_back(0xFFFFFFFFu);
        for (int tid = lo; tid < hi; ++tid) {
            const TemplatePyramid& tp = c.pyramids[tid];
            if ((int)tp.size() != L * M) { err = "template pyramid size mismatch"; return false; }
            const u32 ti = (u32)out.t_global.size();
            out.t_global.push_back(tid);
            out.t_class.push_back(ci);
            const Template& t0 = tp[(size_t)(L - 1) * M];
            int n_total = 0, cnt_packed = 0;
            int P = 0;
            double fcount = 0;
            for (int m = 0; m < M; ++m) {
                const Template& t = tp[(size_t)(L - 1) * M + m];
                n_total += (int)t.features.size();
                if (t.width != t0.width || t.height != t0.height) { err = "modalities of one pyramid level must share width/height"; return false; }
                int wf = (t.width - 1) / gl.T + 1, hf = (t.height - 1) / gl.T + 1;
                const int span_x = gl.W - wf, span_y = gl.H - hf;
                const long long P64 = (long long)span_y * gl.W + span_x + 1;
                P = (int)std::min<long long>(std::max<long long>(P64, 0), (long long)gl.wh);
                int k = 0;
                const size_t list_begin = out.scan_off.size();
                for (const lm_feature& f : t.features) {
                    if (f.x < 0 || f.x >= gl.w || f.y < 0 || f.y >= gl.h) continue;
                    u32 off = osc * ((u32)m * gl.mod_stride + (u32)f.label * gl.ori_stride) +
                              (u32)((f.y % gl.T) * gl.T + (f.x % gl.T)) * gl.wh + (u32)(f.y / gl.T) * gl.W + (u32)(f.x / gl.T);
                    out.scan_off.push_back(off);
                    ++k;
                }
                fcount += k;
                cnt_packed |= k << (8 + 8 * m);
                std::sort(out.scan_off.begin() + (ptrdiff_t)list_begin, out.scan_off.end());
                {
                    const int feat_order = scan_list_order;
                    if (feat_order == 2) std::reverse(out.scan_off.begin() + (ptrdiff_t)list_begin, out.scan_off.end());
                    if (feat_order == 1) {
                        std::vector<std::vector<u32>> by_label(8);
                        for (size_t q = list_begin; q < out.scan_off.size(); ++q) {
                            const u32 rel = out.scan_off[q] / osc - (u32)m * gl.mod_stride;
                            by_label[std::min<u32>(rel / gl.ori_stride, 7u)].push_back(out.scan_off[q]);
                        }
                        size_t q = list_begin;
                        for (size_t r = 0; q < out.scan_off.size(); ++r)
                            for (int lb = 0; lb < 8; ++lb) if (r < by_label[lb].size()) out.scan_off[q++] = by_label[lb][r];
                    }
                    if (feat_order == 3) {
                        struct FP { u32 off; int x, y, lab; };
                        std::vector<FP> fp;
                        for (const lm_feature& f : t.features) {
                            if (f.x < 0 || f.x >= gl.w || f.y < 0 || f.y >= gl.h) continue;
                            const u32 off = osc * ((u32)m * gl.mod_stride + (u32)f.label * gl.ori_stride) +
                                            (u32)((f.y % gl.T) * gl.T + (f.x % gl.T)) * gl.wh + (u32)(f.y / gl.T) * gl.W + (u32)(f.x / gl.T);
                            fp.push_back(FP{off, f.x, f.y, f.label});
                        }
                        std::vector<long> best(fp.size(), (long)1 << 40);
                        std::vector<char> used(fp.size(), 0);
                        size_t cur = 0;
                        for (size_t q = 1; q < fp.size(); ++q) if (fp[q].off < fp[cur].off) cur = q;
                        for (size_t r = 0; r < fp.size(); ++r) {
                            out.scan_off[list_begin + r] = fp[cur].off;
                            used[cur] = 1;
                            size_t nxt = cur; long far = -1;
                            for (size_t q = 0; q < fp.size(); ++q) {
                                if (used[q]) continue;
                                const int dl = std::min((fp[q].lab - fp[cur].lab) & 7, (fp[cur].lab - fp[q].lab) & 7);
                                const long dd = (long)(fp[q].x - fp[cur].x) * (fp[q].x - fp[cur].x) + (long)(fp[q].y - fp[cur].y) * (fp[q].y - fp[cur].y) + 16L * dl * dl;
                                best[q] = std::min(best[q], dd);
                                if (best[q] > far || (best[q] == far && fp[q].off < fp[nxt].off)) { far = best[q]; nxt = q; }
                            }
                            cur = nxt;
                        }
                    }
                }
                for (; k < out.fpad; ++k) out.scan_off.push_back(osc * gl.zero_off);
            }
            if (planes) {
                const size_t b1 = out.off1.size();
                for (int m = 0; m < M; ++m) {
                    const int k = (cnt_packed >> (8 + 8 * m)) & 0xFF;
                    const size_t lb = ((size_t)ti * M + m) * out.fpad;
                    for (int q = 0; q < k; ++q) {
                        const u32 noff = out.scan_off[lb + q];
                        out.offn.push_back(noff); out.off1.push_back(plane_bit_off(noff));
                        const u32 base = noff / 2u, mm = base / gl.mod_stride, label = (base - mm * gl.mod_stride) / gl.ori_stride;
                        out.offs3.push_back((label << 29) | (mm * gl.mod_stride + (noff - 2u * (mm * gl.mod_stride + label * gl.ori_stride))));
                    }
                }
                if (out.lds_ok) {
                    for (size_t q = b1; q < out.off1.size(); ++q) {
                        const u32 e3 = out.offs3[q], label = e3 >> 29, so = e3 & 0x1FFFFFFFu, mm = so / gl.mod_stride, rest = so - mm * gl.mod_stride;
                        const u32 bit = 8u * (mm * 8u + label) * pb + rest;
                        out.offl.push_back((((bit >> 5) << 2) << 8) | (bit & 31u));
                        out.offsl.push_back((label << 29) | (mm * ttwh + rest));
                    }
                    while (out.offl.size() < b1 + (size_t)out.fpad1) { out.offl.push_back(((u32)M * ttwh) << 8); out.offsl.push_back(0u); }
                    out.lbegin.push_back((int)out.litem.size());
                    for (int un = 0; un * 128 < P; ++un) out.litem.push_back((ti << 8) | (u32)un);
                }
                while (out.off1.size() < b1 + (size_t)out.fpad1) { out.offn.push_back(2u * gl.zero_off); out.off1.push_back(8u * gl.zero_off); out.offs3.push_back(gl.zero_off); }
                for (int L1 = 1; L1 <= 64; ++L1) out.items1_by_L[L1] += (P + (128 * L1 - 31) - 1) / (128 * L1 - 31);
            }
            const int chunk = gl.nibble ? LM_SCAN4_CHUNK : LM_SCAN_CHUNK;
            out.scan_P.push_back(P);
            out.scan_n.push_back(n_total | cnt_packed);
            out.class_alg_bytes[ci] += fcount * (double)P;
            out.class_load_bytes[ci] += fcount * (double)((P + chunk - 1) / chunk) * (gl.nibble ? 512.0 : 1024.0);
            for (int ch = 0; ch * chunk < P; ++ch) { out.item_t.push_back(ti); out.item_chunk.push_back((u32)ch); }
            for (int l = 0; l + 1 < L; ++l) {
                const LmLevelGeom& g = geom[l];
                LmRefMeta mt;
                std::memset(&mt, 0, sizeof(mt));
                mt.width = tp[(size_t)l * M].width;
                mt.height = tp[(size_t)l * M].height;
                for (int m = 0; m < M; ++m) {
                    const Template& t = tp[(size_t)l * M + m];
                    mt.nfeat_total += (int)t.features.size();
                    mt.start[m] = (u32)out.ref_feat[l].size();
                    mt.count[m] = (u32)t.features.size();
                    for (const lm_feature& f : t.features) {
                        LmRefFeat rf;
                        rf.off = ((u32)m * g.mod_stride + (u32)((f.y % g.T) * g.T + (f.x % g.T)) * g.wh +
                                  (u32)(f.y / g.T) * g.W + (u32)(f.x / g.T)) |
                                 ((u32)f.label << 29);
                        if ((u64)m * g.mod_stride + (u64)((f.y % g.T) * g.T + (f.x % g.T)) * g.wh + (u64)(f.y / g.T) * g.W +
                                (u64)(f.x / g.T) >= (1ull << 29)) { err = "feature too far outside the frame"; return false; }
                        rf.x = (int16_t)f.x; rf.y = (int16_t)f.y;
                        out.ref_feat[l].push_back(rf);
                    }
                }
                out.ref_meta[l].push_back(mt);
            }
        }
        out.class_t_hi[ci] = (int)out.t_global.size();
        out.class_item_hi[ci] = (int)out.item_t.size();
    }
    if (out.lds_ok) {
        out.lbegin.push_back((int)out.litem.size());
        if (out.t_global.size() >= (1u << (32 - LM_SCANL_POS_BITS)) || out.litem.empty()) out.lds_ok = false;
    }
    if (out.lds_ok) {
        schedule_lds_lists(out);
        out.lrec.assign(out.litem.size() * 4u, 0u);
        for (size_t i = 0; i < out.litem.size(); ++i) {
            const u32 it = out.litem[i];
            out.lrec[4 * i] = it;
            if (it != 0xFFFFFFFFu) { out.lrec[4 * i + 1] = (u32)out.scan_n[it >> 8]; out.lrec[4 * i + 2] = (u32)out.scan_P[it >> 8]; }
        }
    }
    return true;
}

void schedule_lds_lists(DeviceBankHost& out) {
    const size_t nt = out.t_global.size();
    const int fp = out.fpad1;
    auto residue = [](u32 e) { return (int)(((e >> 8) >> 2) & 3u); };
    std::vector<u32> tmp((size_t)fp);
    std::vector<char> used((size_t)fp);
    for (size_t t = 0; t < nt; ++t) {
        const int lb = out.lbegin[t], le = out.lbegin[t + 1];
        int last = le;
        while (last > lb && out.litem[(size_t)last - 1] == 0xFFFFFFFFu) --last;
        if (last <= lb) continue;
        const int g_first = lb / 32;
        std::vector<size_t> nb;
        for (size_t p = t; p-- > 0 && nb.size() < 8;) {
            int pl = out.lbegin[p + 1];
            while (pl > out.lbegin[p] && out.litem[(size_t)pl - 1] == 0xFFFFFFFFu) --pl;
            if (pl <= out.lbegin[p]) continue;
            if ((pl - 1) / 32 < g_first) break;
            nb.push_back(p);
        }
        if (nb.empty()) continue;
        u32* list = out.offl.data() + t * (size_t)fp;
        const int cnt = out.scan_n[t];
        const int nreal = std::min(fp, ((cnt >> 8) & 0xFF) + ((cnt >> 16) & 0xFF));
        std::fill(used.begin(), used.end(), 0);
        for (int k = 0; k < nreal; ++k) {
            bool taken[4] = {false, false, false, false};
            for (size_t p : nb) taken[residue(out.offl[p * (size_t)fp + (size_t)k])] = true;
            int pick = -1, first = -1;
            for (int q = 0; q < nreal; ++q) {
                if (used[(size_t)q]) continue;
                if (first < 0) first = q;
                if (!taken[residue(list[q])]) { pick = q; break; }
            }
            if (pick < 0) pick = first;
            used[(size_t)pick] = 1;
            tmp[(size_t)k] = list[pick];
        }
        for (int k = 0; k < nreal; ++k) list[k] = tmp[(size_t)k];
    }
}

void build_items1(const DeviceBankHost& hb, int L, std::vector<u32>& item_t, std::vector<u32>& item_chunk, std::vector<int>& begin) {
    const int chunk = 128 * L - 31;
    item_t.clear(); item_chunk.clear(); begin.clear();
    for (size_t t = 0; t < hb.scan_P.size(); ++t) {
        begin.push_back((int)item_t.size());
        for (int ch = 0; ch * chunk < hb.scan_P[t]; ++ch) { item_t.push_back((u32)t); item_chunk.push_back((u32)ch); }
    }
    begin.push_back((int)item_t.size());
}

void build_hull_table(const Bank& bank, int M, HullTable& out) {
    out = HullTable();
    struct P { int x, y; };
    std::vector<P> p, hull;
    for (const ClassEntry& c : bank.classes) {
        out.class_base.push_back((u32)out.hull_off.size());
        for (const TemplatePyramid& tp : c.pyramids) {
            out.hull_off.push_back((u32)(out.hull_xy.size() / 2));
            p.clear();
            for (int m = 0; m < M && m < (int)tp.size(); ++m)
                for (const lm_feature& f : tp[(size_t)m].features) p.push_back(P{f.x, f.y});
            std::sort(p.begin(), p.end(), [](const P& a, const P& b) { return a.x < b.x || (a.x == b.x && a.y < b.y); });
            p.erase(std::unique(p.begin(), p.end(), [](const P& a, const P& b) { return a.x == b.x && a.y == b.y; }), p.end());
            if (p.size() >= 3) {
                auto crs = [](const P& o, const P& a, const P& b) { return (long long)(a.x - o.x) * (b.y - o.y) - (long long)(a.y - o.y) * (b.x - o.x); };
                hull.assign(2 * p.size(), P{0, 0});
                size_t k = 0;
                for (size_t i = 0; i < p.size(); ++i) {
                    while (k >= 2 && crs(hull[k - 2], hull[k - 1], p[i]) <= 0) --k;
                    hull[k++] = p[i];
                }
                for (size_t i = p.size() - 1, t = k + 1; i > 0; --i) {
                    while (k >= t && crs(hull[k - 2], hull[k - 1], p[i - 1]) <= 0) --k;
                    hull[k++] = p[i - 1];
                }
                hull.resize(k - 1);
            } else {
                hull = p;
            }
            for (const P& q : hull) { out.hull_xy.push_back((int16_t)q.x); out.hull_xy.push_back((int16_t)q.y); }
        }
    }
    out.hull_off.push_back((u32)(out.hull_xy.size() / 2));
    if (out.class_base.empty()) out.class_base.push_back(0);
}

void default_similarity_lut(u8 lut[256]) {
    static const u8 kUpstream[256] = {
        0, 4, 3, 4, 2, 4, 3, 4, 1, 4, 3, 4, 2, 4, 3, 4,  0, 0, 0, 0, 0, 0, 0, 0, 0, 0, 0, 0, 0, 0, 0, 0,
        0, 3, 4, 4, 3, 3, 4, 4, 2, 3, 4, 4, 3, 3, 4, 4,  0, 1, 0, 1, 0, 1, 0, 1, 0, 1, 0, 1, 0, 1, 0, 1,
        0, 2, 3, 3, 4, 4, 4, 4, 3, 3, 3, 3, 4, 4, 4, 4,  0, 2, 1, 2, 0, 2, 1, 2, 0, 2, 1, 2, 0, 2, 1, 2,
        0, 1, 2, 2, 3, 3, 3, 3, 4, 4, 4, 4, 4, 4, 4, 4,  0, 3, 2, 3, 1, 3, 2, 3, 0, 3, 2, 3, 1, 3, 2, 3,
        0, 0, 1, 1, 2, 2, 2, 2, 3, 3, 3, 3, 3, 3, 3, 3,  0, 4, 3, 4, 2, 4, 3, 4, 1, 4, 3, 4, 2, 4, 3, 4,
        0, 1, 0, 1, 1, 1, 1, 1, 2, 2, 2, 2, 2, 2, 2, 2,  0, 3, 4, 4, 3, 3, 4, 4, 2, 3, 4, 4, 3, 3, 4, 4,
        0, 2, 1, 2, 0, 2, 1, 2, 1, 2, 1, 2, 1, 2, 1, 2,  0, 2, 3, 3, 4, 4, 4, 4, 3, 3, 3, 3, 4, 4, 4, 4,
        0, 3, 2, 3, 1, 3, 2, 3, 0, 3, 2, 3, 1, 3, 2, 3,  0, 1, 2, 2, 3, 3, 3, 3, 4, 4, 4, 4, 4, 4, 4, 4};
    std::memcpy(lut, kUpstream, 256);
}

void default_normal_lut(u8 lut[8000]) {
    const double PI = 3.14159265358979323846;
    for (int v3 = 0; v3 < 20; ++v3)
        for (int v2 = 0; v2 < 20; ++v2)
            for (int v1 = 0; v1 < 20; ++v1) {
                double nx = (v1 + 0.5 - 10.0) / 10.0, ny = (v2 + 0.5 - 10.0) / 10.0;
                double a = std::atan2(ny, nx);
                if (a < 0) a += 2 * PI;
                int bin = (int)std::floor(a / (PI / 4.0));
                if (bin > 7) bin = 7;
                lut[v3 * 400 + v2 * 20 + v1] = (u8)(1u << bin);
            }
}

bool match_less(const lm_match_t& a, const lm_match_t& b) {
    if (a.similarity != b.similarity) return a.similarity > b.similarity;
    if (a.template_id != b.template_id) return a.template_id < b.template_id;
    if (a.class_idx != b.class_idx) return a.class_idx < b.class_idx;
    if (a.y != b.y) return a.y < b.y;
    return a.x < b.x;
}
bool match_eq(const lm_match_t& a, const lm_match_t& b) {
    return a.x == b.x && a.y == b.y && a.similarity == b.similarity && a.class_idx == b.class_idx;
}
void sort_unique(std::vector<lm_match_t>& v) {
    std::sort(v.begin(), v.end(), match_less);
    v.erase(std::unique(v.begin(), v.end(), match_eq), v.end());
}

namespace {
// ... 188 lines not shown
```

line-mod-pipeline_amd/csrc/lm_host.h:

```cpp
#pragma once
#include <string>
#include <vector>

#include "../../include/linemod_hip.h"
#include "lm_common.h"

namespace lmh {

struct Template {
    int width = 0, height = 0, pyramid_level = 0;
    std::vector<lm_feature> features;
};
typedef std::vector<Template> TemplatePyramid;

struct ClassEntry {
    std::string id;
    std::vector<TemplatePyramid> pyramids;
};

struct Bank {
    std::vector<ClassEntry> classes;
    int find(const std::string& id) const;
    int add_class(const std::string& id, int n_templates, const lm_template_desc* descs, const lm_feature* features,
                  int levels, int modalities, std::string& err);
    int add_pyramid(const std::string& id, TemplatePyramid&& tp);
};

bool check_template_pyramid(const TemplatePyramid& tp, int levels, int modalities, std::string& err);
bool check_modality_params(const lm_config& cfg, std::string& err);

struct DeviceBankHost {
    int fpad = LM_SCAN_FPAD;
    std::vector<int> t_global, t_class;
    std::vector<u32> scan_off;
    std::vector<int> scan_P, scan_n;
    std::vector<u32> item_t, item_chunk;
    std::vector<int> class_item_lo, class_item_hi;
    std::vector<int> class_t_lo, class_t_hi;
    std::vector<double> class_alg_bytes;
    std::vector<double> class_load_bytes;
    std::vector<LmRefMeta> ref_meta[LM_MAX_LEVELS];
    std::vector<LmRefFeat> ref_feat[LM_MAX_LEVELS];
    int fpad1 = 0;
    std::vector<u32> off1, offn, offs3;
    long long items1_by_L[65] = {};
    bool lds_ok = false;
    std::vector<u32> offl;
    std::vector<u32> offsl;
    std::vector<u32> litem;
    std::vector<u32> lrec;
    std::vector<int> lbegin;
};
void build_items1(const DeviceBankHost& hb, int L, std::vector<u32>& item_t, std::vector<u32>& item_chunk, std::vector<int>& begin);
bool lds_image_fits(const LmLevelGeom& g, int M);

enum class Layout : unsigned char {
    Responses,
    ResponsesAndPlanes,
    SpreadAndPlanes,
};
inline unsigned layout_bit(Layout l) { return 1u << (unsigned)l; }
inline bool layouts_mixed(unsigned held) {
    return (held & layout_bit(Layout::SpreadAndPlanes)) && held != layout_bit(Layout::SpreadAndPlanes);
}

struct ScanInputs {
    int form = 0;
    int M = 1;
    bool nibble = false, planes = false;
    bool lds_fits = false;
    bool bank_built = false;
    bool scanl_bank = false;
    bool scanl_device = false;
    int fpad1 = 0;
    const long long* items1_by_L = nullptr;
    long long items4 = 0;
    size_t frame_stride = 0;
    u32 arena_bytes = 0;
    float threshold = -1.0f;
    float scan1_min_threshold = 50.0f;
    int scanl_min_slots = 24;
    int scanl_R = 0;
};

Layout plan_layout(const ScanInputs& in, int n);

struct ScanPlan {
    enum Kind {
        Scan4,
        Scan1,
        ScanL,
        Mixed,
        NoBitPlaneForm,
    };
    Kind kind = Scan4;
    int param = 0;
};
ScanPlan plan_scan(const ScanInputs& in, int nslots, unsigned layouts, int n_litems);

inline void shard_range(int n, int rank, int size, int* lo, int* hi) {
    *lo = (int)((long long)n * rank / size);
    *hi = (int)((long long)n * (rank + 1) / size);
}

bool build_device_bank(const Bank& bank, const lm_config& cfg, const LmLevelGeom* geom, DeviceBankHost& out,
                       int scan_list_order, std::string& err);

struct HullTable {
    std::vector<u32> class_base;
    std::vector<u32> hull_off;
    std::vector<int16_t> hull_xy;
};
void build_hull_table(const Bank& bank, int modalities, HullTable& out);

void default_similarity_lut(u8 lut[256]);
void default_normal_lut(u8 lut[8000]);

bool match_less(const lm_match_t& a, const lm_match_t& b);
bool match_eq(const lm_match_t& a, const lm_match_t& b);
void sort_unique(std::vector<lm_match_t>& v);

bool save_bank(const Bank& bank, const lm_config& cfg, const char* path, std::string& err);
bool load_bank(Bank& bank, const lm_config& cfg, const char* path, std::string& err);


void copy_stream(void* dst, const void* src, size_t n);
void copy_stream_fence();

struct ShiftRect { int x0, x1, y0, y1; };
ShiftRect shift_rect(int w, int h, int ox, int oy);
inline int clamp_shift(int v, int extent) { return v < -extent ? -extent : (v > extent ? extent : v); }
void stage_rows_shifted(u8* staging, const u8* src, size_t stride, int w, int h, int px, int ox, int oy, int r0, int r1);
}
```

line-mod-pipeline_amd/csrc/lm_k_refine.hip:

```cpp
#include "lm_dev.h"

namespace {


__device__ __forceinline__ void emit_key(const LmRefineArgs& a, LmDevHeader* hdr, u64* keys, u32 ti, int x, int y,
                                         float sim) {
    u32 slot = atomicAdd(&hdr->match_count, 1u);
    if (slot < a.match_cap) {
        u32 sb = __float_as_uint(sim);
        u64 hi = ((u64)(~sb) << 32) | (u32)a.t_global[ti];
        u64 lo = ((u64)(u32)a.t_class[ti] << 48) | ((u64)((u32)(y + 0x800000) & 0xFFFFFFu) << 24) |
                 (u64)((u32)(x + 0x800000) & 0xFFFFFFu);
        keys[2 * (size_t)slot] = hi;
        keys[2 * (size_t)slot + 1] = lo;
    }
}

#define RP_MAXP 1056
__global__ __launch_bounds__(1024) void k_refine_plan(const LmDevHeader* __restrict__ hdr0, size_t aux_slot_stride,
                                                       int nslots, u32 cand_cap, int cap, u32* __restrict__ plan) {
    __shared__ u32 cnt[RP_MAXP], pslot[RP_MAXP], poff[RP_MAXP];
    __shared__ u32 sorted_cnt[RP_MAXP], sorted_piece[RP_MAXP];
    __shared__ u32 pl[8 * 136 * 3 + 16 + 8];
    __shared__ u32 wsum[16], wbase[17];
    const int tid = threadIdx.x, lane = tid & 63, wv = tid >> 6;
    u32 c = 0;
    if (tid < nslots) {
        c = slot_ptr_s(hdr0, aux_slot_stride, (u32)tid)->cand_count;
        if (c > cand_cap) c = cand_cap;
    }
    u32 t = c;
#pragma unroll
    for (int o = 32; o >= 1; o >>= 1) t += (u32)__shfl_xor((int)t, o, 64);
    if (lane == 0) wsum[wv] = t;
    __syncthreads();
    u32 total = 0;
#pragma unroll
    for (int k = 0; k < 16; ++k) total += wsum[k];
    const u32 P = max(64u, ((total + 23u) / 24u + 1u) & ~1u);
    const u32 np = tid < nslots ? max(1u, (c + P - 1u) / P) : 0u;
    u32 inc = np;
#pragma unroll
    for (int o = 1; o < 64; o <<= 1) { const u32 v = (u32)__shfl_up((int)inc, o, 64); if (lane >= o) inc += v; }
    __syncthreads();
    if (lane == 63) wsum[wv] = inc;
    __syncthreads();
    if (tid == 0) { u32 acc = 0; for (int k = 0; k < 16; ++k) { wbase[k] = acc; acc += wsum[k]; } wbase[16] = acc; }
    __syncthreads();
    const u32 NP = wbase[16];
    const u32 pbase = wbase[wv] + inc - np;
    for (u32 k = 0; k < np; ++k) { cnt[pbase + k] = min(P, c - k * P); pslot[pbase + k] = (u32)tid; poff[pbase + k] = k * P; }
    if (np == 1 && c == 0) cnt[pbase] = 0;
    __syncthreads();
    for (u32 e = (u32)tid; e < NP; e += 1024u) {
        const u32 ce = cnt[e];
        u32 rank = 0;
#pragma unroll 8
        for (u32 j = 0; j < NP; ++j) {
            const u32 cj = cnt[j];
            rank += (cj > ce || (cj == ce && j < e)) ? 1u : 0u;
        }
        sorted_cnt[rank] = ce; sorted_piece[rank] = e;
    }
    __syncthreads();
    if (tid < 64) {
        const u32 x = (u32)tid & 7u;
        u32 load = 0, len = 0;
        u32 rc[2], rs[2];
#pragma unroll
        for (int q = 0; q < 2; ++q) { rc[q] = sorted_cnt[(tid + 64 * q) % RP_MAXP]; rs[q] = sorted_piece[(tid + 64 * q) % RP_MAXP]; }
        for (u32 r = 0; r < NP; ++r) {
            u32 sc, ss;
            if (r < 128) {
                const int src = (int)(r & 63u);
                sc = (u32)__builtin_amdgcn_readlane((int)(r < 64 ? rc[0] : rc[1]), src);
                ss = (u32)__builtin_amdgcn_readlane((int)(r < 64 ? rs[0] : rs[1]), src);
            } else {
                sc = sorted_cnt[r]; ss = sorted_piece[r];
            }
            u32 key = (int)len < cap ? ((load << 3) | x) : 0xFFFFFFFFu;
            key = min(key, (u32)__builtin_amdgcn_mov_dpp((int)key, 0xB1, 0xf, 0xf, true));
            key = min(key, (u32)__builtin_amdgcn_mov_dpp((int)key, 0x4E, 0xf, 0xf, true));
            key = min(key, (u32)__builtin_amdgcn_mov_dpp((int)key, 0x141, 0xf, 0xf, true));
            if ((key & 7u) == x) {
                if (tid < 8) pl[x * cap + len] = ss;
                len += 1; load += sc + 8u;
            }
        }
        if (tid < 8) pl[8 * cap + x] = len;
    }
    __syncthreads();
    if (tid < 8) {
        u32 acc = 0;
        u32* pre = pl + 8 * cap + 8 + tid * (cap + 1);
        u32* off = pl + 8 * cap + 8 + 8 * (cap + 1) + tid * cap;
        const u32 n = pl[8 * cap + tid];
        for (u32 k = 0; k < n; ++k) {
            const u32 pc = pl[tid * cap + k];
            pre[k] = acc; acc += cnt[pc];
            off[k] = poff[pc];
            pl[tid * cap + k] = pslot[pc];
        }
        for (u32 k = n; k <= (u32)cap; ++k) pre[k] = acc;
        for (u32 k = n; k < (u32)cap; ++k) off[k] = 0;
    }
    __syncthreads();
    for (int i = tid; i < 8 * cap + 8 + 8 * (cap + 1) + 8 * cap; i += 1024) plan[i] = pl[i];
}

#define PRUNE_REFINE true
#ifndef PRUNE_REFINE_PAIR
#define PRUNE_REFINE_PAIR false
#endif
template <bool W4>
__device__ __forceinline__ u32 rf_patch(const u8* __restrict__ lm, u32 se, u32 lane_off) {
    if (W4) {
        const u32x2 d = ld8a4(lm + ((se & ~3u) + lane_off));
        return __builtin_amdgcn_alignbyte(d[1], d[0], se);
    }
    const u32 t = se + lane_off;
    const u32x2 d = ld8a4(lm + (t & ~3u));
    return __builtin_amdgcn_alignbyte(d[1], d[0], t);
}
__device__ __forceinline__ void rf_lookup(const u8* __restrict__ tab, u32 v, u32 (&r)[4]) {
    r[0] = tab[v & 0xFFu]; r[1] = tab[(v >> 8) & 0xFFu]; r[2] = tab[(v >> 16) & 0xFFu]; r[3] = tab[v >> 24];
}
template <bool LAST, bool W4>
__device__ __forceinline__ void refine_one(const LmRefineArgs& a, u32 slot, u32 i, const u8 (*resp)[256], int lane) {
    LmDevHeader* hdr = slot_ptr_s(a.hdr, a.aux_slot_stride, slot);
    LmCand* cand = slot_ptr_s(a.cand, a.aux_slot_stride, slot);
    u64* keys = slot_ptr_s(a.keys, a.aux_slot_stride, slot);
    const u8* lm = a.lm + (size_t)slot * a.lm_slot_stride;
    const int T = a.g.T, W = a.g.W;
    const int border = 8 * T;
    const int offset = T / 2 + (T % 2 - 1);
    const u32 lane_off = (u32)((lane >> 2) * W + (lane & 3) * 4);
    LmCand c = cand[i];
    u32 ti = (u32)__builtin_amdgcn_readfirstlane((int)c.ti);
    if (ti == LM_DROPPED) return;
    int cx = __builtin_amdgcn_readfirstlane(c.x), cy = __builtin_amdgcn_readfirstlane(c.y);
    const LmRefMeta mt = a.meta[ti];
    int max_x = a.g.w - mt.width - border, max_y = a.g.h - mt.height - border;
    int x = cx * 2 + 1, y = cy * 2 + 1;
    x = x > border ? x : border; y = y > border ? y : border;
    x = x < max_x ? x : max_x;  y = y < max_y ? y : max_y;
    int bx = x / T - 8, by = y / T - 8;
    int off_x = bx * T, off_y = by * T;
    const u32 shift = (u32)(by * W + bx);
    u32 s[4] = {0, 0, 0, 0};
    if (a.stat && lane == 0) atomicAdd(&a.stat[0], 1ull);
    int f_left = mt.nfeat_total;
    const float denom = (float)(4 * mt.nfeat_total);
    bool dead = false;
    for (int m = 0; m < a.M && !dead; ++m) {
        const int cnt = (int)(m == 0 ? mt.count[0] : mt.count[1]);
        const u32 fstart = m == 0 ? mt.start[0] : mt.start[1];
        LmRefFeat ft;
        ft.off = 0; ft.x = 0; ft.y = 0;
        if (lane < cnt) ft = a.feats[fstart + lane];
        int fx = ft.x + off_x, fy = ft.y + off_y;
        bool ok = (lane < cnt) && fx >= 0 && fy >= 0 && fx < a.g.w && fy < a.g.h;
        const u32 eff = ok ? (ft.off & 0x1FFFFFFFu) + shift : a.g.zero_off;
        const u32 lab = ft.off >> 29;
        for (int f = 0; f < cnt; f += 8) {
            u32 v[8], q[8][4];
#pragma unroll
            for (int k = 0; k < 8; ++k) v[k] = rf_patch<W4>(lm, (u32)__builtin_amdgcn_readlane((int)eff, f + k), lane_off);
#pragma unroll
            for (int k = 0; k < 8; ++k) rf_lookup(resp[(u32)__builtin_amdgcn_readlane((int)lab, f + k)], v[k], q[k]);
#pragma unroll
            for (int k = 0; k < 8; k += 2) { s[0] += q[k][0] + q[k + 1][0]; s[1] += q[k][1] + q[k + 1][1]; s[2] += q[k][2] + q[k + 1][2]; s[3] += q[k][3] + q[k + 1][3]; }
            f_left -= min(8, cnt - f);
            if (PRUNE_REFINE && (f & 8) && f_left > 0) {
                const u32 best_now = wave_max_u32(max(max(s[0], s[1]), max(s[2], s[3])));
                const float reach = __fdiv_rn(__fmul_rn((float)(int)(best_now + 4u * (u32)f_left), 100.f), denom);
                if (reach < a.threshold) { dead = true; break; }
            }
        }
    }
    if (dead) {
        if (lane == 0) cand[i].ti = LM_DROPPED;
        if (a.stat && lane == 0) atomicAdd(&a.stat[4], 1ull);
        return;
    }
    u32 idx0 = (u32)lane * 4u;
    u32 k0 = (s[0] << 8) | (255u - idx0);
    u32 k1 = (s[1] << 8) | (254u - idx0);
    u32 k2 = (s[2] << 8) | (253u - idx0);
    u32 k3 = (s[3] << 8) | (252u - idx0);
    u32 k01 = k0 > k1 ? k0 : k1, k23 = k2 > k3 ? k2 : k3;
    u32 key = wave_max_u32(k01 > k23 ? k01 : k23);
    int best = (int)(key >> 8);
    int best_r = -1, best_c = -1;
    if (best > 0) { int idx = 255 - (int)(key & 255u); best_r = idx >> 4; best_c = idx & 15; }
    int nx = (bx + best_c) * T + offset, ny = (by + best_r) * T + offset;
    float sim = __fdiv_rn(__fmul_rn((float)best, 100.f), (float)(4 * mt.nfeat_total));
    if (lane == 0) {
        if (sim < a.threshold) {
            if (a.stat) atomicAdd(&a.stat[5], 1ull);
            cand[i].ti = LM_DROPPED;
        } else if (LAST) {
            emit_key(a, hdr, keys, ti, nx, ny, sim);
        } else {
            LmCand o; o.ti = ti; o.x = nx; o.y = ny; o.sim = sim;
            cand[i] = o;
        }
    }
}

#ifndef RP_BATCH
#define RP_BATCH 8
#endif
static_assert(RP_BATCH % 2 == 0, "the responses are added two features at a time (v_add3_u32)");
template <bool LAST, bool W4>
__device__ __forceinline__ void refine_pair(const LmRefineArgs& a, u32 slot, u32 i, const u8 (*resp)[256], int lane) {
    LmCand* cand = slot_ptr_s(a.cand, a.aux_slot_stride, slot);
    const u32 tiA = (u32)__builtin_amdgcn_readfirstlane((int)cand[i].ti);
    const u32 tiB = (u32)__builtin_amdgcn_readfirstlane((int)cand[i + 1].ti);
    if (tiA != tiB || tiA == LM_DROPPED) {
        refine_one<LAST, W4>(a, slot, i, resp, lane);
        refine_one<LAST, W4>(a, slot, i + 1, resp, lane);
        return;
    }
    LmDevHeader* hdr = slot_ptr_s(a.hdr, a.aux_slot_stride, slot);
    u64* keys = slot_ptr_s(a.keys, a.aux_slot_stride, slot);
    const u8* lm = a.lm + (size_t)slot * a.lm_slot_stride;
    const int T = a.g.T, W = a.g.W;
    const int border = 8 * T;
    const int offset = T / 2 + (T % 2 - 1);
    const u32 lane_off = (u32)((lane >> 2) * W + (lane & 3) * 4);
    const u32 ti = tiA;
    const LmRefMeta mt = a.meta[ti];
    const int max_x = a.g.w - mt.width - border, max_y = a.g.h - mt.height - border;
    int bx[2], by[2], off_x[2], off_y[2];
    u32 shift[2];
#pragma unroll
    for (int c = 0; c < 2; ++c) {
        const LmCand cd = cand[i + c];
        const int cx = __builtin_amdgcn_readfirstlane(cd.x), cy = __builtin_amdgcn_readfirstlane(cd.y);
        int x = cx * 2 + 1, y = cy * 2 + 1;
        x = x > border ? x : border; y = y > border ? y : border;
        x = x < max_x ? x : max_x;  y = y < max_y ? y : max_y;
        bx[c] = x / T - 8; by[c] = y / T - 8;
        off_x[c] = bx[c] * T; off_y[c] = by[c] * T;
        shift[c] = (u32)(by[c] * W + bx[c]);
    }
    u32 s[2][4] = {{0, 0, 0, 0}, {0, 0, 0, 0}};
    if (a.stat && lane == 0) atomicAdd(&a.stat[1], 2ull);
    const int dcol = bx[1] - bx[0];
    const bool same_rows = by[0] == by[1] && dcol >= 0 && dcol <= 4;
    int f_left = mt.nfeat_total;
    const float denom = (float)(4 * mt.nfeat_total);
    for (int m = 0; m < a.M; ++m) {
        const int cnt = (int)(m == 0 ? mt.count[0] : mt.count[1]);
        const u32 fstart = m == 0 ? mt.start[0] : mt.start[1];
        LmRefFeat ft;
        ft.off = 0; ft.x = 0; ft.y = 0;
        if (lane < cnt) ft = a.feats[fstart + lane];
        u32 eff[2];
        bool ok2[2];
#pragma unroll
        for (int c = 0; c < 2; ++c) {
            const int fx = ft.x + off_x[c], fy = ft.y + off_y[c];
            const bool ok = (lane < cnt) && fx >= 0 && fy >= 0 && fx < a.g.w && fy < a.g.h;
            ok2[c] = ok;
            eff[c] = ok ? (ft.off & 0x1FFFFFFFu) + shift[c] : a.g.zero_off;
        }
        const u32 lab = ft.off >> 29;
        const bool share = W4 && same_rows && __all(lane >= cnt || (ok2[0] && ok2[1]));
        for (int f = 0; f < cnt; f += RP_BATCH) {
            u32 v[2][RP_BATCH], q[2][RP_BATCH][4];
            if (share) {
#pragma unroll
                for (int k = 0; k < RP_BATCH; ++k) {
                    const u32 se = (u32)__builtin_amdgcn_readlane((int)eff[0], f + k);
                    u32 d0, d1, d2;
                    ld12a4(lm + ((se & ~3u) + lane_off), d0, d1, d2);
                    const u32 o = (se & 3u) + (u32)dcol;
                    const bool up = o >= 4u;
                    v[0][k] = __builtin_amdgcn_alignbyte(d1, d0, se);
                    v[1][k] = __builtin_amdgcn_alignbyte(up ? d2 : d1, up ? d1 : d0, o);
                }
            } else {
#pragma unroll
            for (int k = 0; k < RP_BATCH; ++k)
#pragma unroll
                for (int c = 0; c < 2; ++c) v[c][k] = rf_patch<W4>(lm, (u32)__builtin_amdgcn_readlane((int)eff[c], f + k), lane_off);
            }
#pragma unroll
            for (int k = 0; k < RP_BATCH; ++k) {
                const u8* tab = resp[(u32)__builtin_amdgcn_readlane((int)lab, f + k)];
#pragma unroll
                for (int c = 0; c < 2; ++c) rf_lookup(tab, v[c][k], q[c][k]);
            }
#pragma unroll
            for (int k = 0; k < RP_BATCH; k += 2)
#pragma unroll
                for (int c = 0; c < 2; ++c)
#pragma unroll
                    for (int p4 = 0; p4 < 4; ++p4) s[c][p4] += q[c][k][p4] + q[c][k + 1][p4];
            f_left -= min(RP_BATCH, cnt - f);
            if (PRUNE_REFINE_PAIR && (f & RP_BATCH) && f_left > 0) {
                bool out[2];
#pragma unroll
                for (int c = 0; c < 2; ++c) {
                    const u32 best_now = wave_max_u32(max(max(s[c][0], s[c][1]), max(s[c][2], s[c][3])));
                    out[c] = __fdiv_rn(__fmul_rn((float)(int)(best_now + 4u * (u32)f_left), 100.f), denom) < a.threshold;
                }
                if (out[0] || out[1]) {
                    if (a.stat && lane == 0) { atomicAdd(&a.stat[2], (unsigned long long)(out[0] + out[1])); if (out[0] && out[1]) atomicAdd(&a.stat[3], 1ull); }
                    if (out[0] && lane == 0) cand[i].ti = LM_DROPPED;
                    if (out[1] && lane == 0) cand[i + 1].ti = LM_DROPPED;
                    if (!out[0]) refine_one<LAST, W4>(a, slot, i, resp, lane);
                    if (!out[1]) refine_one<LAST, W4>(a, slot, i + 1, resp, lane);
                    return;
                }
            }
        }
    }
#pragma unroll
    for (int c = 0; c < 2; ++c) {
        const u32 idx0 = (u32)lane * 4u;
        const u32 k0 = (s[c][0] << 8) | (255u - idx0), k1 = (s[c][1] << 8) | (254u - idx0);
        const u32 k2 = (s[c][2] << 8) | (253u - idx0), k3 = (s[c][3] << 8) | (252u - idx0);
        const u32 k01 = k0 > k1 ? k0 : k1, k23 = k2 > k3 ? k2 : k3;
        const u32 key = wave_max_u32(k01 > k23 ? k01 : k23);
        const int best = (int)(key >> 8);
        int best_r = -1, best_c = -1;
        if (best > 0) { const int idx = 255 - (int)(key & 255u); best_r = idx >> 4; best_c = idx & 15; }
        const int nx = (bx[c] + best_c) * T + offset, ny = (by[c] + best_r) * T + offset;
        const float sim = __fdiv_rn(__fmul_rn((float)best, 100.f), (float)(4 * mt.nfeat_total));
        if (lane == 0) {
            if (sim < a.threshold) {
                if (a.stat) atomicAdd(&a.stat[5], 1ull);
                cand[i + c].ti = LM_DROPPED;
            } else if (LAST) {
                emit_key(a, hdr, keys, ti, nx, ny, sim);
            } else {
                LmCand o; o.ti = ti; o.x = nx; o.y = ny; o.sim = sim;
                cand[i + c] = o;
            }
        }
    }
}

template <bool LAST, bool W4>
__global__ __launch_bounds__(256) void k_refine(LmRefineArgs a) {
    __shared__ u8 resp[8][256];
    const int lane = threadIdx.x & 63;
    u32 slot = 0, tile = 0, total = 0;
    const u32* xs = nullptr; const u32* xpre = nullptr; const u32* xoff = nullptr;
    u32 xlen = 0;
    if (a.plan) {
        const u32 x = blockIdx.x & 7u;
        tile = blockIdx.x >> 3;
        xs = a.plan + (size_t)x * a.plan_cap;
        xlen = a.plan[(size_t)8 * a.plan_cap + x];
        xpre = a.plan + (size_t)8 * a.plan_cap + 8 + (size_t)x * (a.plan_cap + 1);
        xoff = a.plan + (size_t)8 * a.plan_cap + 8 + (size_t)8 * (a.plan_cap + 1) + (size_t)x * a.plan_cap;
        total = xpre[xlen];
        if (tile * 8u >= total) return;
    } else {
        xcd_slot_tile((u32)a.blocks_per_slot, (u32)a.nslots, slot, tile);
        total = slot_ptr_s(a.hdr, a.aux_slot_stride, slot)->cand_count;
        if (total > a.cand_cap) total = a.cand_cap;
        if (tile * (total <= (u32)a.blocks_per_slot * 4u ? 4u : 8u) >= total) return;
    }
    {
        const u8* sl = reinterpret_cast<const u8*>(a.sim_lut);
        const int v = threadIdx.x;
#pragma unroll
        for (int o = 0; o < 8; ++o) {
            const u8 lo = sl[32 * o + (v & 15)], hi = sl[32 * o + 16 + (v >> 4)];
            resp[o][v] = lo > hi ? lo : hi;
        }
    }
    __syncthreads();
    const u32 wave0 = (u32)__builtin_amdgcn_readfirstlane((int)((tile * 256u + threadIdx.x) >> 6));
    const u32 nwaves = (u32)a.blocks_per_slot * 4u;
    if (a.plan) {
        u32 idx = 0;
        for (u32 g = 2u * wave0; g < total; g += 2u * nwaves) {
            while (idx + 1 < xlen && xpre[idx + 1] <= g) ++idx;
            const u32 i = g - xpre[idx] + xoff[idx];
            if (g + 1 < xpre[idx + 1]) {
                refine_pair<LAST, W4>(a, xs[idx], i, resp, lane);
            } else {
                refine_one<LAST, W4>(a, xs[idx], i, resp, lane);
                if (g + 1 < total) {
                    u32 idx2 = idx;
                    while (idx2 + 1 < xlen && xpre[idx2 + 1] <= g + 1) ++idx2;
                    refine_one<LAST, W4>(a, xs[idx2], g + 1 - xpre[idx2] + xoff[idx2], resp, lane);
                }
            }
        }
    } else if (total <= nwaves) {
        if (wave0 < total) refine_one<LAST, W4>(a, slot, wave0, resp, lane);
    } else {
        for (u32 i = 2u * wave0; i < total; i += 2u * nwaves) {
            if (i + 1 < total) refine_pair<LAST, W4>(a, slot, i, resp, lane);
            else refine_one<LAST, W4>(a, slot, i, resp, lane);
        }
    }
}

__global__ __launch_bounds__(256) void k_emit_unrefined(LmRefineArgs a) {
    LmDevHeader* hdr = slot_ptr(a.hdr, a.aux_slot_stride);
    LmCand* cand = slot_ptr(a.cand, a.aux_slot_stride);
    u64* keys = slot_ptr(a.keys, a.aux_slot_stride);
    u32 n = hdr->cand_count;
    if (n > a.cand_cap) n = a.cand_cap;
    for (u32 i = blockIdx.x * 256u + threadIdx.x; i < n; i += gridDim.x * 256u) {
        LmCand c = cand[i];
        if (c.ti != LM_DROPPED) emit_key(a, hdr, keys, c.ti, c.x, c.y, c.sim);
    }
}

__device__ __forceinline__ void sort_bitonic_lds(u64* hi, u64* lo, u32 N, int tid) {
    bool local_pending = false;
    for (u32 k = 2; k <= N; k <<= 1)
        for (u32 j = k >> 1; j > 0; j >>= 1) {
            if (j > 64 && local_pending) { __syncthreads(); local_pending = false; }
            for (u32 t = tid; t < (N >> 1); t += 1024) {
                u32 i = ((t & ~(j - 1)) << 1) | (t & (j - 1));
                u32 p = i | j;
                bool up = (i & k) == 0;
                u64 ah = hi[i], al = lo[i], bh = hi[p], bl = lo[p];
                bool gt = ah > bh || (ah == bh && al > bl);
                if (gt == up) { hi[i] = bh; lo[i] = bl; hi[p] = ah; lo[p] = al; }
            }
            if (j > 64) __syncthreads();
            else { __builtin_amdgcn_wave_barrier(); local_pending = true; }
        }
    __syncthreads();
}

__device__ __forceinline__ void sort_unique_publish(const u64* hi, const u64* lo, u32 n, u32* wave_tot, LmDevHeader* hdr, LmOutMatch* out,
                                                    LmHostBlock* hb, u32 cand_count, u32 match_count, int tid) {
    u32 base = 0;
    for (u32 c0 = 0; c0 < n; c0 += 1024) {
        u32 i = c0 + tid;
        u32 keep = 0;
        if (i < n) keep = (i == 0) || !(lo[i] == lo[i - 1] && (hi[i] >> 32) == (hi[i - 1] >> 32));
        unsigned long long bal = __ballot(keep);
        int lane = tid & 63, wv = tid >> 6;
        u32 pre = __popcll(bal & ((1ull << lane) - 1ull));
        if (lane == 0) wave_tot[wv] = __popcll(bal);
        __syncthreads();
        u32 woff = 0, tot = 0;
        for (int k = 0; k < 16; ++k) { u32 t = wave_tot[k]; if (k < wv) woff += t; tot += t; }
        if (keep) {
            u64 h = hi[i], l = lo[i];
            LmOutMatch m;
            m.similarity = __uint_as_float(~(u32)(h >> 32));
            m.template_id = (int)(u32)h;
            m.class_idx = (int)(l >> 48);
            m.y = (int)((l >> 24) & 0xFFFFFFu) - 0x800000;
            m.x = (int)(l & 0xFFFFFFu) - 0x800000;
            u32 pos = base + woff + pre;
            out[pos] = m;
            if (pos < LM_INLINE_MATCHES) hb->rec[pos] = m;
        }
        base += tot;
        __syncthreads();
    }
    if (tid == 0) {
        hb->hdr.cand_count = cand_count; hb->hdr.match_count = match_count;
        hb->hdr.out_count = base; hb->hdr.sorted_on_device = 1;
        hdr->pad[0] = base;
    }
}

__global__ __launch_bounds__(1024) void k_sort_unique(LmSortArgs a) {
    extern __shared__ __attribute__((aligned(16))) u8 smem[];
    u64* hi = reinterpret_cast<u64*>(smem);
    u64* lo = hi + LM_SORT_CAP;
    __shared__ u32 wave_tot[16];
    LmDevHeader* hdr = slot_ptr(a.hdr, a.aux_slot_stride);
    u64* keys = slot_ptr(a.keys, a.aux_slot_stride);
    LmOutMatch* out = slot_ptr(a.out, a.aux_slot_stride);
    LmHostBlock* hb = reinterpret_cast<LmHostBlock*>(reinterpret_cast<u8*>(a.host) + (size_t)blockIdx.z * a.host_slot_stride);
    const int tid = threadIdx.x;
    const u32 chunk = blockIdx.y;
    const u32 cand_count = hdr->cand_count, match_count = hdr->match_count;
    u32 n = match_count;
    if (n > a.match_cap) n = a.match_cap;
    __syncthreads();
    const bool unsortable = n > LM_SORT_CAP || cand_count > a.cand_cap || match_count > a.match_cap;
    if (a.split && !unsortable && n > LM_SORT_CHUNK) {
        const u32 c0 = chunk * LM_SORT_CHUNK;
        if (c0 >= n) return;
        const u32 cnt = min(n - c0, (u32)LM_SORT_CHUNK);
        u32 N = 64;
        while (N < cnt) N <<= 1;
        for (u32 i = tid; i < N; i += 1024) {
            hi[i] = i < cnt ? keys[2 * (size_t)(c0 + i)] : ~0ull;
            lo[i] = i < cnt ? keys[2 * (size_t)(c0 + i) + 1] : ~0ull;
        }
        __syncthreads();
        sort_bitonic_lds(hi, lo, N, tid);
        for (u32 i = tid; i < cnt; i += 1024) { keys[2 * (size_t)(c0 + i)] = hi[i]; keys[2 * (size_t)(c0 + i) + 1] = lo[i]; }
        return;
    }
    if (chunk != 0) return;
    if (tid == 0) { hdr->cand_count = 0; hdr->match_count = 0; }
    if (unsortable) {
        if (tid == 0) {
            hb->hdr.cand_count = cand_count; hb->hdr.match_count = match_count;
            hb->hdr.out_count = 0; hb->hdr.sorted_on_device = 0;
            hdr->pad[0] = (cand_count > a.cand_cap || match_count > a.match_cap) ? 0xFFFFFFFEu : 0xFFFFFFFFu;
        }
        return;
    }
    if (n <= 256) {
        __shared__ u32 rk[1024];
        u64 mh = ~0ull, ml = ~0ull;
        if ((u32)tid < n) { mh = keys[2 * (size_t)tid]; ml = keys[2 * (size_t)tid + 1]; }
        hi[tid] = mh; lo[tid] = ml;
        rk[tid] = 0;
        __syncthreads();
        u32 n2 = 64;
        while (n2 < n) n2 <<= 1;
        const u32 teams = 1024u / n2, e = (u32)tid & (n2 - 1u), team = (u32)tid / n2;
        const u64 eh = hi[e], el = lo[e];
        const u32 j0 = (u32)((u64)n * team / teams), j1 = (u32)((u64)n * (team + 1u) / teams);
        u32 rank = 0;
        if (e < n) {
#pragma unroll 8
            for (u32 j = j0; j < j1; ++j) {
                const u64 h = hi[j], l = lo[j];
                const bool before = h < eh || (h == eh && (l < el || (l == el && j < e)));
                rank += before ? 1u : 0u;
            }
            if (teams > 1) atomicAdd(&rk[e], rank);
            else rk[e] = rank;
        }
        __syncthreads();
        const u32 myrank = rk[tid];
        __syncthreads();
        if ((u32)tid < n) { hi[myrank] = mh; lo[myrank] = ml; }
        __syncthreads();
    } else {
        u32 N = 1;
        while (N < n) N <<= 1;
        for (u32 i = tid; i < N; i += 1024) {
            hi[i] = i < n ? keys[2 * (size_t)i] : ~0ull;
            lo[i] = i < n ? keys[2 * (size_t)i + 1] : ~0ull;
        }
        __syncthreads();
        sort_bitonic_lds(hi, lo, N, tid);
    }
    sort_unique_publish(hi, lo, n, wave_tot, hdr, out, hb, cand_count, match_count, tid);
}

__global__ __launch_bounds__(1024) void k_merge_unique(LmSortArgs a) {
    extern __shared__ __attribute__((aligned(16))) u8 smem[];
    u64* hi = reinterpret_cast<u64*>(smem);
    u64* lo = hi + LM_SORT_CAP;
    __shared__ u32 wave_tot[16];
    LmDevHeader* hdr = slot_ptr(a.hdr, a.aux_slot_stride);
    const u64* keys = slot_ptr(a.keys, a.aux_slot_stride);
    LmOutMatch* out = slot_ptr(a.out, a.aux_slot_stride);
    LmHostBlock* hb = reinterpret_cast<LmHostBlock*>(reinterpret_cast<u8*>(a.host) + (size_t)blockIdx.z * a.host_slot_stride);
    const int tid = threadIdx.x;
    const u32 cand_count = hdr->cand_count, match_count = hdr->match_count;
    const u32 n = match_count;
    __syncthreads();
    if (n <= LM_SORT_CHUNK || n > LM_SORT_CAP || cand_count > a.cand_cap || match_count > a.match_cap) return;
    if (tid == 0) { hdr->cand_count = 0; hdr->match_count = 0; }
    for (u32 i = tid; i < n; i += 1024) { hi[i] = keys[2 * (size_t)i]; lo[i] = keys[2 * (size_t)i + 1]; }
    __syncthreads();
    constexpr int PER = LM_SORT_CAP / 1024;
    u64 eh[PER], el[PER];
    u32 rank[PER];
#pragma unroll
    for (int k = 0; k < PER; ++k) {
        const u32 i = (u32)tid + 1024u * (u32)k;
        rank[k] = 0xFFFFFFFFu;
        if (i >= n) continue;
        eh[k] = hi[i]; el[k] = lo[i];
        const u32 c = i / LM_SORT_CHUNK;
        u32 r = i - c * LM_SORT_CHUNK;
        for (u32 b = 0; b < n; b += LM_SORT_CHUNK) {
            if (b == c * LM_SORT_CHUNK) continue;
            const u32 len = min(n - b, (u32)LM_SORT_CHUNK);
            const bool earlier = b < c * LM_SORT_CHUNK;
            u32 pos = 0;
#pragma unroll
            for (u32 step = LM_SORT_CHUNK; step >= 1; step >>= 1) {
                const u32 q = pos + step;
                if (q <= len) {
                    const u64 h = hi[b + q - 1], l = lo[b + q - 1];
                    const bool before = h < eh[k] || (h == eh[k] && (earlier ? l <= el[k] : l < el[k]));
                    pos = before ? q : pos;
                }
            }
            r += pos;
        }
        rank[k] = r;
    }
    __syncthreads();
#pragma unroll
    for (int k = 0; k < PER; ++k)
        if (rank[k] != 0xFFFFFFFFu) { hi[rank[k]] = eh[k]; lo[rank[k]] = el[k]; }
    __syncthreads();
    sort_unique_publish(hi, lo, n, wave_tot, hdr, out, hb, cand_count, match_count, tid);
}

__global__ __launch_bounds__(256) void k_pack_lists(LmPackArgs a) {
    __shared__ u32 part[4];
    const int tid = threadIdx.x, slot = blockIdx.x;
    u32 s = 0;
    for (int j = tid; j < slot; j += 256) {
        const u32 c = slot_ptr_s(a.hdr, a.aux_slot_stride, (u32)j)->pad[0];
        s += c >= 0xFFFFFFFEu ? 0u : c;
    }
#pragma unroll
    for (int o = 32; o >= 1; o >>= 1) s += (u32)__shfl_xor((int)s, o, 64);
    if ((tid & 63) == 0) part[tid >> 6] = s;
    __syncthreads();
    const u32 prefix = part[0] + part[1] + part[2] + part[3];
    u32 mine = slot_ptr_s(a.hdr, a.aux_slot_stride, (u32)slot)->pad[0];
    if (mine >= 0xFFFFFFFEu) { if (tid == 0) atomicOr(reinterpret_cast<u32*>(a.cnt + a.nslots), mine == 0xFFFFFFFEu ? 4u : 2u); mine = 0; }
    if (tid == 0) a.cnt[slot] = (int)mine;
    if (prefix + mine > a.cap_total) { if (tid == 0) atomicOr(reinterpret_cast<u32*>(a.cnt + a.nslots), 1u); return; }
    const u32* src = reinterpret_cast<const u32*>(slot_ptr_s(a.out, a.aux_slot_stride, (u32)slot));
    u32* dst = reinterpret_cast<u32*>(a.rec) + (size_t)prefix * 5;
    for (u32 i = tid; i < mine * 5u; i += 256) dst[i] = src[i];
}



}

void lmk_refine_plan(hipStream_t s, const LmRefineArgs& a, int nslots, u32* plan, int plan_cap) {
    hipLaunchKernelGGL(k_refine_plan, dim3(1), dim3(1024), 0, s, a.hdr, a.aux_slot_stride, nslots, a.cand_cap, plan_cap, plan);
}

void lmk_refine(hipStream_t s, const LmRefineArgs& a_in, bool last, int nslots) {
    LmRefineArgs a = a_in;
    a.blocks_per_slot = 256; a.nslots = nslots;
    dim3 grid(a.plan ? (unsigned)(8 * a.blocks_per_slot) : (unsigned)(a.blocks_per_slot * nslots), 1, 1);
    const bool w4 = (a.g.W & 3) == 0;
    if (last) { if (w4) hipLaunchKernelGGL((k_refine<true, true>), grid, dim3(256), 0, s, a); else hipLaunchKernelGGL((k_refine<true, false>), grid, dim3(256), 0, s, a); }
    else { if (w4) hipLaunchKernelGGL((k_refine<false, true>), grid, dim3(256), 0, s, a); else hipLaunchKernelGGL((k_refine<false, false>), grid, dim3(256), 0, s, a); }
}

void lmk_emit_unrefined(hipStream_t s, const LmRefineArgs& a, int nslots) {
    hipLaunchKernelGGL(k_emit_unrefined, dim3(64, 1, nslots), dim3(256), 0, s, a);
}

void lmk_pack_lists(hipStream_t s, const LmPackArgs& a) {
    (void)hipMemsetAsync(a.cnt + a.nslots, 0, sizeof(int), s);
    hipLaunchKernelGGL(k_pack_lists, dim3((unsigned)a.nslots), dim3(256), 0, s, a);
}

void lmk_sort_unique(hipStream_t s, const LmSortArgs& a, int nslots) {
    size_t shmem = (size_t)LM_SORT_CAP * 16;
    hipLaunchKernelGGL(k_sort_unique, dim3(1, a.split ? LM_SORT_CAP / LM_SORT_CHUNK : 1, nslots), dim3(1024), shmem, s, a);
    if (a.split) hipLaunchKernelGGL(k_merge_unique, dim3(1, 1, nslots), dim3(1024), shmem, s, a);
}
```

line-mod-pipeline_amd/csrc/lm_kernels.h:

```cpp
#pragma once
#include <hip/hip_runtime.h>
#include "lm_common.h"

void lmk_pyrdown(hipStream_t s, const u8* src, int sw, int sh, u8* dst, size_t slot_stride, int nslots);
void lmk_set_pyrdown_variant(int v);
void lmk_nn_half(hipStream_t s, const u8* src, int src_pitch, u8* dst, int dw, int dh, size_t slot_stride, int nslots);
size_t lmk_color_scratch_bytes(int w, int h);
void lmk_set_cgrad_variant(int v);
void lmk_set_cblur_variant(int v);
void lmk_color_quantize(hipStream_t s, const u8* bgr, int w, int h, float weak_threshold, u8* quant, float* mag,
                        u8* scratch, size_t slot_stride, int nslots, bool blurred = false);
bool lmk_blur_pyrdown(hipStream_t s, const u8* bgr0, int w, int h, u8* scratch0, u8* bgr1, u8* quant0, size_t slot_stride, int nslots);
bool lmk_color_blur(hipStream_t s, const u8* bgr, int w, int h, u8* scratch, size_t slot_stride, int nslots);
bool lmk_cgrad_levels_wanted(int w0, int h0, int nslots);
bool lmk_cgrad_levels(hipStream_t s, const u8* S0, int w0, int h0, u8* q0, const u8* S1, int w1, int h1, u8* q1, float weak_threshold, size_t slot_stride, int nslots);
void lmk_set_cgrad_levels(int v);
void lmk_set_blur_pyr(int v);
void lmk_set_blur_pyr_interleave(int v);
void lmk_set_slot_weight(int w);
void lmk_set_blur_strip(int v);
void lmk_depth_quantize(hipStream_t s, const u16* depth, int w, int h, int dist_thr, int diff_thr, const u8* lut,
                        bool lut_onehot, u8* quant, u8* scratch, size_t slot_stride, int nslots);
bool lmk_nibble_supported(int w, int h, int T);
void lmk_linear_memories(hipStream_t s, const u8* q, int qpitch, int src_shift, int mode, int w, int h, int T,
                         const u64* resp_tab, u8* lm, u32 ori_stride, size_t q_slot_stride, size_t lm_slot_stride,
                         int nslots, u32 plane_ori = 0);

#define LM_MASK_SLOTS 128
#define LM_MASK_LEVELS 4
struct LmMaskArgs {
    u8* frame;
    size_t slot_stride;
    u32 off_quant[LM_MASK_LEVELS][2];
    u32 w[LM_MASK_LEVELS];
    u32 vec_begin[LM_MASK_LEVELS + 1];
    u32 vec_depth;
    u32 mask_pitch;
    int levels;
    int vec_rows;
    int n;
    u16 slot[LM_MASK_SLOTS];
    const u8* cmask[LM_MASK_SLOTS];
    const u8* dmask[LM_MASK_SLOTS];
};
void lmk_match_mask(hipStream_t s, const LmMaskArgs& a);

#define LM_RULE_KINDS 8
#define LM_RULE_MAX_GROW 16
struct LmHsvRange { int lo[3], hi[3]; };
struct LmRule {
    LmHsvRange hsv;
    int use_depth, keep_invalid, use_hsv;
    int zmin, zmax;
    int grow;
    int rx, ry, rw, rh;
};
struct LmRuleArgs {
    const u8* bgr; const u16* depth;
    size_t slot_stride;
    const int* divtab;
    int w, h;
    u32 mask_pitch;
    int rows_out;
    int vec;
    int n;
    LmRule rule[LM_RULE_KINDS];
    u16 slot[LM_MASK_SLOTS];
    u8 kind[LM_MASK_SLOTS];
    u8* plane[LM_MASK_SLOTS];
};
bool lmk_mask_rule_fits(int w);
void lmk_mask_rule(hipStream_t s, LmRuleArgs& a);

struct LmScanArgs {
    const u8* lm;
    size_t lm_slot_stride;
    const u32* item_t;
    const u32* item_chunk;
    int item_lo, n_items;
    int nibble;
    const u32* scan_off;
    const int* scan_P;
    const int* scan_n;
    int M, fpad;
    const int* raw_thr_by_n;
    int W, T;
    LmDevHeader* hdr;
    LmCand* cand;
    size_t aux_slot_stride;
    u32 cand_cap;
    unsigned long long* stat;
    int wgs_per_slot, nslots;
    int L1, G1;
    u32 L1_rcp16;
    u32 delta_rcp16;
    const u32* off1;
    const u32* offn;
    int fpad1;
    int no_exact;
    unsigned long long* surv;
    u32 surv_cap;
    int surv_set;
    int exact_spread;
    const u32* offs3;
    const u64* resp_tab;
    int lds_form, R;
    const u32* offl;
    const u32* offsl;
    const u32* litem;
    int litem_lo, n_litems;
    u32 pb;
    u32 mod_stride, planes_off, plane_ori;
    u32 tbl_bytes;
    u32 queue_cap;
    int dbg;
};
#define LM_SCAN_VARIANT_SETTABLE (0x3F | 0x100)
void lmk_scan(hipStream_t s, const LmScanArgs& a, int variant, int nslots);
bool lmk_scanl_raise_lds();

struct LmRefineArgs {
    const u8* lm;
    size_t lm_slot_stride;
    LmLevelGeom g;
    int M;
    const LmRefMeta* meta;
    const LmRefFeat* feats;
    const u32* sim_lut;
    LmDevHeader* hdr;
    LmCand* cand;
    u64* keys;
    size_t aux_slot_stride;
    u32 cand_cap;
    u32 match_cap;
    float threshold;
    const int* t_global;
    const int* t_class;
    const u32* plan;
    int plan_cap;
    int blocks_per_slot, nslots;
    unsigned long long* stat;
};
void lmk_refine_plan(hipStream_t s, const LmRefineArgs& a, int nslots, u32* plan, int plan_cap);
void lmk_refine(hipStream_t s, const LmRefineArgs& a, bool last, int nslots);
void lmk_emit_unrefined(hipStream_t s, const LmRefineArgs& a, int nslots);

struct LmSortArgs {
    LmDevHeader* hdr;
    u64* keys;
    LmOutMatch* out;
    size_t aux_slot_stride;
    LmHostBlock* host;
    size_t host_slot_stride;
    u32 cand_cap, match_cap;
    int split;
};
void lmk_sort_unique(hipStream_t s, const LmSortArgs& a, int nslots);

struct LmPackArgs {
    const LmDevHeader* hdr;
    const LmOutMatch* out;
    size_t aux_slot_stride;
    int nslots;
    u32 cap_total;
    int* cnt;
    LmOutMatch* rec;
};
void lmk_pack_lists(hipStream_t s, const LmPackArgs& a);

#define LM_HULL_MAX 128
void lmk_hsv_mask(hipStream_t s, const u8* bgr, int w, int h, const LmHsvRange& rg, const int* divtab, u32* mask, int wpr,
                  size_t in_stride, size_t mask_stride, int nslots);
#define LMK_NORMAL_CODE_OFFSET 8000
struct LmPhaseArgs {
    const u8* bgr0; u8* bgr1; const u16* depth;
    u8 *cs0, *cs1, *ds;
    u8 *qc0, *qc1, *qd0;
    u8 *lm_c0, *lm_c1, *lm_d0, *lm_d1;
    int w, h;
    float weak_threshold; int dist_thr, diff_thr;
    const u8* normal_lut; const u64* resp_tab;
    u32 ori_stride1;
    u32 plane_ori1;
    size_t slot_stride; int nslots;
};
bool lmk_phases_supported(const LmPhaseArgs& a, int T0, int T1, int mode0, int mode1, bool lut_onehot);
void lmk_preprocess_phases(hipStream_t s, const LmPhaseArgs& a, int T0);
bool lmk_batch_phases_supported(const LmPhaseArgs& a, int T0, int T1, int mode0, int mode1, bool lut_onehot);
void lmk_preprocess_batch_phases(hipStream_t s, const LmPhaseArgs& a, int T0);
void lmk_set_dmedian_variant(int v);
void lmk_selftest_float_tail(hipStream_t s, unsigned long long* out2);

struct LmHullArgs {
    const LmOutMatch* matches; u32 n;
    const u32* class_base;
    const u32* hull_off;
    const int16_t* hull_xy;
    const u32* mask; int wpr;
    const int* match_slot;
    size_t mask_slot_words;
    int w, h;
    long long* out;
};
bool lmk_hull_counts(hipStream_t s, const LmHullArgs& a);

struct LmDepthQuery { int x0, y0, x1, y1; int lo, hi; int slot; int pad; };
struct LmDepthArgs {
    const u16* depth;
    size_t slot_stride;
    int w, h;
    const LmDepthQuery* q; u32 n;
    u32* out;
};
void lmk_depth_counts(hipStream_t s, const LmDepthArgs& a);

struct LmIcpSceneScratch { u32* z; unsigned long long* zsum; u32* blockcnt; u32* blockoff; u32* counts; };
void lmk_icp_scene(hipStream_t st, const u16* depth, int W, int H, int x0, int y0, int bw, int bh, float fx, float fy, float cx, float cy,
                   int step, LmIcpSceneScratch sc, float* out);
struct LmIcpPose {
    double P[12];
    double pose[12];
    double posex[12];
    double mean_avg[3], scale;
    double fval_old, fval_perc, thr;
    int it, done;
};
struct LmIcpNN { double d; int j; int pad; };
struct LmIcpLevel { int level, s, nL, ndL, rounds, max_it; double tolp; };
struct LmIcpScratch { LmIcpPose* st; double* src0; double* srcL; LmIcpNN* part; float* nd; int* nidx; unsigned long long* keys; double* acc; };
int lmk_icp_nn_chunks(int ndL);
void lmk_icp_register(hipStream_t st, const float* model, int nm, const float* scene, int ns, int np, const LmIcpLevel* levels, int nlevels,
                      double rejection_scale, LmIcpScratch w, double* out);

void lmk_icp_verify(hipStream_t s, bool from_z, const void* renders, const u16* scenes, const int* scene_idx, size_t scene_stride, int nq, int w,
                    int h, int scene_min, u32* out);

struct LmGenCand { int16_t x, y; int32_t label; float score; };
struct LmGenGeom {
    int L, M, rows;
    int w[4], h[4], et[4];
    size_t off[4], img_px;
    size_t q_off[4][2], mag_off[4];
    float min_mag;
};
void lmk_gen_render(hipStream_t s, const float* xyz, int nv, const u32* idx, int ntri, const float* vp, int nviews, int W, int H,
                    float4* sv, u32* zbuf, u8* cov, u16* depth);
void lmk_gen_zbuffer(hipStream_t s, const float* xyz, int nv, const u32* idx, int ntri, const float* vp, int nviews, int W, int H,
                     float4* sv, u32* zbuf);
void lmk_gen_rotate(hipStream_t s, const u8* cov, const u16* dep, const int* img_view, const int* img_angle, const int* tabs, int nimg,
                    int W, int H, u8* rmask, u16* rdepth, u8* bgr_slot, u16* depth_slot, size_t slot_stride, u8* er);
void lmk_gen_candidates(hipStream_t s, int pass, const u8* er, int W, int H, int nimg, const LmGenGeom& g, u8* flags, u16* hp,
                        const u8* slot0, const u8* mag, size_t slot_stride, u32* cnt, u32* icnt, const u32* rowoff, LmGenCand* out);

void lmk_eval_vsd(hipStream_t s, bool from_z, const void* renders, const u16* scenes, const int* scene_idx, int nq, size_t npx, int delta,
                  int tau, u32* counts);
size_t lmk_eval_add_parts(int m);
void lmk_eval_add(hipStream_t s, const float* xyz, int step, int m, const float* queries, int nq, int symmetric, float4* gt, float4* est,
                  u32* minbits, float* dist, double* part, float* mean);
```

Measured before the change: 198,400.

## Store spread memories in 32-column strips with apron for refine patch loads

Changes the spread-only linear memory layout from row-major W-pitch planes to 32-column strips with a 64-byte row pitch. Each strip keeps a duplicated apron of the next columns, so the 16x16 refine patch reads become fixed-pitch aligned loads regardless of W. Refine feature offsets now encode only the memory plane, and the row and column are computed per candidate using a reciprocal divide. A separate wrap-path kernel variant handles templates whose patches exceed the frame. The cost is extra duplicate stores in the spread kernels, more arena memory, and more index arithmetic in refine.

```diff
diff --git a/line-mod-pipeline_amd/csrc/lm_common.h b/line-mod-pipeline_amd/csrc/lm_common.h
--- a/line-mod-pipeline_amd/csrc/lm_common.h
+++ b/line-mod-pipeline_amd/csrc/lm_common.h
@@ -17,6 +17,18 @@
 #define LM_SORT_CHUNK 1024
 #define LM_INLINE_MATCHES 2048
 #define LM_DROPPED 0xFFFFFFFFu
+
+#define LM_STRIP_COLS 32
+#define LM_STRIP_PITCH 64
+#if defined(__HIPCC__) || defined(__CUDACC__)
+#define LM_HD __host__ __device__
+#else
+#define LM_HD
+#endif
+LM_HD inline u32 lm_strip_count(int W) { return ((u32)W + LM_STRIP_COLS - 1u) / LM_STRIP_COLS; }
+LM_HD inline u32 lm_strip_bytes(int H) { return (u32)H * LM_STRIP_PITCH; }
+LM_HD inline u32 lm_strip_mem_bytes(int W, int H) { return lm_strip_count(W) * lm_strip_bytes(H); }
+LM_HD inline u32 lm_strip_off(int H, int r, int c) { return ((u32)c >> 5) * lm_strip_bytes(H) + (u32)r * LM_STRIP_PITCH + ((u32)c & 31u); }
 
 struct LmLevelGeom {
     int w, h;
@@ -48,6 +60,7 @@
     int nfeat_total;
     u32 start[2];
     u32 count[2];
+    u32 qmax;
 };
 
 struct LmDevHeader {
diff --git a/line-mod-pipeline_amd/csrc/lm_detector.hip b/line-mod-pipeline_amd/csrc/lm_detector.hip
--- a/line-mod-pipeline_amd/csrc/lm_detector.hip
+++ b/line-mod-pipeline_amd/csrc/lm_detector.hip
@@ -533,6 +533,7 @@
     a.g = d->geom[level];
     a.M = d->cfg.num_modalities;
     a.meta = d->d_ref_meta[level]; a.feats = d->d_ref_feat[level];
+    a.wrap = d->hb.ref_wraps[level] ? 1 : 0;
     a.sim_lut = d->d_sim_lut;
     a.hdr = reinterpret_cast<LmDevHeader*>(d->aux(first, d->off_hdr));
     a.cand = reinterpret_cast<LmCand*>(d->aux(first, d->off_cand));
@@ -829,7 +830,12 @@
         size_t ori = align_up(((size_t)T * T * g.wh) >> g.nibble, 256) + pad;
         size_t plane = g.nibble ? align_up(((size_t)T * T * g.wh + 7) / 8 + ((size_t)g.wh + 64 * 128) / 8 + 64, 256) : 0;
         if (g.nibble && (size_t)c.num_modalities * (8 * ori + 8 * plane) + pad > 0x1FFFFFFFull) plane = 0;
-        size_t mod = g.spread_only ? ori : 8 * ori + 8 * plane;
+        size_t mod = 8 * ori + 8 * plane;
+        if (g.spread_only) {
+            mod = align_up((size_t)T * T * lm_strip_mem_bytes(g.W, g.H), 256);
+            ori = mod;
+            pad = align_up(16 * (size_t)LM_STRIP_PITCH + 64, 256);
+        }
         size_t arena = (size_t)c.num_modalities * mod + pad;
         if (arena > (g.spread_only ? 0x1FFFFFFFull : g.nibble ? 0x7FFFFFFFull : 0xFFFFFFFFull)) { delete d; return fail(LM_ERR_INVALID, "frame too large for the arena offset encoding"); }
         g.ori_stride = (u32)ori;
diff --git a/line-mod-pipeline_amd/csrc/lm_detector_debug.hip b/line-mod-pipeline_amd/csrc/lm_detector_debug.hip
--- a/line-mod-pipeline_amd/csrc/lm_detector_debug.hip
+++ b/line-mod-pipeline_amd/csrc/lm_detector_debug.hip
@@ -115,6 +115,20 @@
     return LM_OK;
 }
 
+static int read_spread_logical(lm_detector* d, int slot, int level, int modality, u8* out) {
+    const LmLevelGeom& g = d->geom[level];
+    const size_t blk = (size_t)g.T * g.T * g.wh;
+    const u8* src = d->lm(slot, level) + (size_t)modality * g.mod_stride;
+    if (!g.spread_only) { HIP_TRY(hipMemcpy(out, src, blk, hipMemcpyDeviceToHost)); return LM_OK; }
+    const size_t ms = lm_strip_mem_bytes(g.W, g.H);
+    std::vector<u8> raw((size_t)g.T * g.T * ms);
+    HIP_TRY(hipMemcpy(raw.data(), src, raw.size(), hipMemcpyDeviceToHost));
+    for (int mem = 0; mem < g.T * g.T; ++mem)
+        for (int r = 0; r < g.H; ++r)
+            for (int c = 0; c < g.W; ++c) out[(size_t)mem * g.wh + (size_t)r * g.W + c] = raw[(size_t)mem * ms + lm_strip_off(g.H, r, c)];
+    return LM_OK;
+}
+
 int lm_debug_read(lm_detector* d, int slot, int what, int level, int modality, uint8_t* out, size_t cap, size_t* size_out) {
     int rc;
     if ((rc = ready_for_compute(d))) return rc;
@@ -140,6 +154,16 @@
         if (size_out) *size_out = blk;
         if (out) {
             if (cap < blk) return fail(LM_ERR_INVALID, "buffer too small");
+            if ((rc = read_spread_logical(d, slot, level, modality, out))) return rc;
+        }
+        return LM_OK;
+    }
+    if (what == 3) {
+        size_t blk = (size_t)g.T * g.T * lm_strip_mem_bytes(g.W, g.H);
+        if (!g.spread_only) return fail(LM_ERR_INVALID, "the lowest level keeps response memories, not the spread memory");
+        if (size_out) *size_out = blk;
+        if (out) {
+            if (cap < blk) return fail(LM_ERR_INVALID, "buffer too small");
             HIP_TRY(hipMemcpy(out, d->lm(slot, level) + (size_t)modality * g.mod_stride, blk, hipMemcpyDeviceToHost));
         }
         return LM_OK;
@@ -152,7 +176,7 @@
             if (cap < n) return fail(LM_ERR_INVALID, "buffer too small");
             if (g.spread_only || (level == d->cfg.pyramid_levels - 1 && d->slots[slot].layout == lmh::Layout::SpreadAndPlanes)) {
                 std::vector<u8> sp(blk);
-                HIP_TRY(hipMemcpy(sp.data(), d->lm(slot, level) + (size_t)modality * g.mod_stride, blk, hipMemcpyDeviceToHost));
+                if ((rc = read_spread_logical(d, slot, level, modality, sp.data()))) return rc;
                 for (int o = 0; o < 8; ++o)
                     for (size_t i = 0; i < blk; ++i)
                         out[o * blk + i] = std::max(d->sim_lut[32 * o + (sp[i] & 15)], d->sim_lut[32 * o + 16 + (sp[i] >> 4)]);
diff --git a/line-mod-pipeline_amd/csrc/lm_dev_memories.h b/line-mod-pipeline_amd/csrc/lm_dev_memories.h
--- a/line-mod-pipeline_amd/csrc/lm_dev_memories.h
+++ b/line-mod-pipeline_amd/csrc/lm_dev_memories.h
@@ -2,6 +2,13 @@
 #include "lm_dev.h"
 
 namespace {
+
+template <class V>
+__device__ __forceinline__ void strip_store(u8* __restrict__ mem, int H, int r, int c, V v) {
+    u8* p = mem + lm_strip_off(H, r, c);
+    *reinterpret_cast<V*>(p) = v;
+    if (c >= LM_STRIP_COLS) *reinterpret_cast<V*>(p - lm_strip_bytes(H) + LM_STRIP_COLS) = v;
+}
 
 #define LMK_MAX_LOADS 8
 template <int SRC_SHIFT, bool SPREAD_ONLY>
@@ -14,6 +21,7 @@
     u8* lm = slot_ptr(lm0, lm_slot_stride);
     const int W = w / T;
     const u32 wh = (u32)W * (u32)(h / T);
+    const u32 ms = lm_strip_mem_bytes(W, h / T);
     const int rows = 2 * T - 1;
     const int pitch = (seg * T + T + 3) & ~3;
     u64* tab = reinterpret_cast<u64*>(smem);
@@ -73,7 +81,7 @@
             }
             u8* dst = lm + (size_t)g * wh + (size_t)band * W + col0 + 4 * k4;
             if (SPREAD_ONLY) {
-                *reinterpret_cast<u32*>(dst) = (u32)sv[0] | ((u32)sv[1] << 8) | ((u32)sv[2] << 16) | ((u32)sv[3] << 24);
+                strip_store<u32>(lm + (size_t)g * ms, h / T, band, col0 + 4 * k4, (u32)sv[0] | ((u32)sv[1] << 8) | ((u32)sv[2] << 16) | ((u32)sv[3] << 24));
             } else {
                 u64 e0 = tab[sv[0]], e1 = tab[sv[1]], e2 = tab[sv[2]], e3 = tab[sv[3]];
 #pragma unroll
@@ -94,7 +102,7 @@
             for (int r = 0; r < T; ++r) sv |= p[r * pitch];
             u8* dst = lm + (size_t)g * wh + (size_t)band * W + col0 + k;
             if (SPREAD_ONLY) {
-                dst[0] = sv;
+                strip_store<u8>(lm + (size_t)g * ms, h / T, band, col0 + k, sv);
             } else {
                 u64 e = tab[sv];
 #pragma unroll
@@ -274,7 +282,7 @@
         const u32 s2 = row[(4 * k4 + 2) * T + c0], s3 = row[(4 * k4 + 3) * T + c0];
         u8* dst = lm + (size_t)g * wh + (size_t)band * W + col0 + 4 * k4;
         if (SPREAD_ONLY) {
-            *reinterpret_cast<u32*>(dst) = s0 | (s1 << 8) | (s2 << 16) | (s3 << 24);
+            strip_store<u32>(lm + (size_t)g * lm_strip_mem_bytes(W, h / T), h / T, band, col0 + 4 * k4, s0 | (s1 << 8) | (s2 << 16) | (s3 << 24));
         } else {
             const u64 e0 = tab[s0], e1 = tab[s1], e2 = tab[s2], e3 = tab[s3];
             const u32 a0 = (u32)e0, a1 = (u32)e1, a2 = (u32)e2, a3 = (u32)e3;
@@ -307,7 +315,7 @@
     const u8* q = slot_ptr_s(q0, q_slot_stride, slot);
     u8* lm = slot_ptr_s(lm0, lm_slot_stride, slot);
     const int ng = w >> 5, W = w >> 1;
-    const u32 wh = (u32)W * (u32)(h >> 1);
+    const u32 ms = lm_strip_mem_bytes(W, h >> 1);
     const int gid = (int)(tile * 256u) + (int)threadIdx.x;
     const int yp = gid / ng, g = gid - yp * ng;
     const int y = 2 * yp;
@@ -338,9 +346,9 @@
             od[k] = __builtin_amdgcn_perm(sp[2 * k + 1], sp[2 * k], 0x07050301u);
         }
         if (y + r < h) {
-            u8* base = lm + (size_t)(2 * r) * wh + (size_t)yp * W + 16 * g;
-            st16(base, u32x4{ev[0], ev[1], ev[2], ev[3]});
-            st16(base + wh, u32x4{od[0], od[1], od[2], od[3]});
+            u8* mem = lm + (size_t)(2 * r) * ms;
+            strip_store<u32x4>(mem, h >> 1, yp, 16 * g, u32x4{ev[0], ev[1], ev[2], ev[3]});
+            strip_store<u32x4>(mem + ms, h >> 1, yp, 16 * g, u32x4{od[0], od[1], od[2], od[3]});
         }
     }
 }
@@ -362,7 +370,7 @@
     const u8* q = slot_ptr_s(q0, q_slot_stride, slot);
     u8* lm = slot_ptr_s(lm0, lm_slot_stride, slot);
     const int W = w / 5, HB = h / 5, ng = W >> 3;
-    const u32 wh = (u32)W * (u32)HB;
+    const u32 ms = lm_strip_mem_bytes(W, HB);
     const int gid = (int)(tile * 256u) + (int)threadIdx.x;
     const int band = gid / ng, g = gid - band * ng;
     if (band >= HB) return;
@@ -391,10 +399,14 @@
         u32 V[11];
 #pragma unroll
         for (int d = 0; d < 11; ++d) V[d] = Hr[j][d] | Hr[j + 1][d] | Hr[j + 2][d] | Hr[j + 3][d] | Hr[j + 4][d];
-        u8* dst = lm + (size_t)(j * 5) * wh + (size_t)band * W + 8 * g;
-#pragma unroll
-        for (int c0 = 0; c0 < 5; ++c0)
-            *reinterpret_cast<u32x2*>(dst + (size_t)c0 * wh) = u32x2{gather4_stride5(V, c0), gather4_stride5(V, c0 + 20)};
+        u8* dst = lm + (size_t)(j * 5) * ms + lm_strip_off(HB, band, 8 * g);
+        const bool apron = 8 * g >= LM_STRIP_COLS;
+#pragma unroll
+        for (int c0 = 0; c0 < 5; ++c0) {
+            const u32x2 v = u32x2{gather4_stride5(V, c0), gather4_stride5(V, c0 + 20)};
+            *reinterpret_cast<u32x2*>(dst + (size_t)c0 * ms) = v;
+            if (apron) *reinterpret_cast<u32x2*>(dst + (size_t)c0 * ms - lm_strip_bytes(HB) + LM_STRIP_COLS) = v;
+        }
     }
 }
 __global__ __launch_bounds__(256) void k_lm_spread5(const u8* __restrict__ q0, int qpitch, int w, int h, u8* __restrict__ lm0,
diff --git a/line-mod-pipeline_amd/csrc/lm_host.cpp b/line-mod-pipeline_amd/csrc/lm_host.cpp
--- a/line-mod-pipeline_amd/csrc/lm_host.cpp
+++ b/line-mod-pipeline_amd/csrc/lm_host.cpp
@@ -243,6 +243,7 @@
                 std::memset(&mt, 0, sizeof(mt));
                 mt.width = tp[(size_t)l * M].width;
                 mt.height = tp[(size_t)l * M].height;
+                u32 qmax_x = 0, qmax_y = 0;
                 for (int m = 0; m < M; ++m) {
                     const Template& t = tp[(size_t)l * M + m];
                     mt.nfeat_total += (int)t.features.size();
@@ -250,15 +251,17 @@
                     mt.count[m] = (u32)t.features.size();
                     for (const lm_feature& f : t.features) {
                         LmRefFeat rf;
-                        rf.off = ((u32)m * g.mod_stride + (u32)((f.y % g.T) * g.T + (f.x % g.T)) * g.wh +
-                                  (u32)(f.y / g.T) * g.W + (u32)(f.x / g.T)) |
-                                 ((u32)f.label << 29);
-                        if ((u64)m * g.mod_stride + (u64)((f.y % g.T) * g.T + (f.x % g.T)) * g.wh + (u64)(f.y / g.T) * g.W +
-                                (u64)(f.x / g.T) >= (1ull << 29)) { err = "feature too far outside the frame"; return false; }
+                        const u64 mem_off = (u64)m * g.mod_stride + (u64)((f.y % g.T) * g.T + (f.x % g.T)) * lm_strip_mem_bytes(g.W, g.H);
+                        if (mem_off + lm_strip_mem_bytes(g.W, g.H) > (1ull << 29)) { err = "feature too far outside the frame"; return false; }
+                        rf.off = (u32)mem_off | ((u32)f.label << 29);
+                        qmax_x = std::max(qmax_x, (u32)(f.x / g.T)); qmax_y = std::max(qmax_y, (u32)(f.y / g.T));
                         rf.x = (int16_t)f.x; rf.y = (int16_t)f.y;
                         out.ref_feat[l].push_back(rf);
                     }
                 }
+                mt.qmax = std::min(qmax_x, 0xFFFFu) | (std::min(qmax_y, 0xFFFFu) << 16);
+                const int bxm = (g.w - mt.width - 8 * g.T) / g.T - 8, bym = (g.h - mt.height - 8 * g.T) / g.T - 8;
+                if (bxm + (int)(mt.qmax & 0xFFFFu) + 16 > g.W || bym + (int)(mt.qmax >> 16) + 16 > g.H) out.ref_wraps[l] = true;
                 out.ref_meta[l].push_back(mt);
             }
         }
diff --git a/line-mod-pipeline_amd/csrc/lm_host.h b/line-mod-pipeline_amd/csrc/lm_host.h
--- a/line-mod-pipeline_amd/csrc/lm_host.h
+++ b/line-mod-pipeline_amd/csrc/lm_host.h
@@ -41,6 +41,7 @@
     std::vector<double> class_load_bytes;
     std::vector<LmRefMeta> ref_meta[LM_MAX_LEVELS];
     std::vector<LmRefFeat> ref_feat[LM_MAX_LEVELS];
+    bool ref_wraps[LM_MAX_LEVELS] = {};
     int fpad1 = 0;
     std::vector<u32> off1, offn, offs3;
     long long items1_by_L[65] = {};
diff --git a/line-mod-pipeline_amd/csrc/lm_k_refine.hip b/line-mod-pipeline_amd/csrc/lm_k_refine.hip
--- a/line-mod-pipeline_amd/csrc/lm_k_refine.hip
+++ b/line-mod-pipeline_amd/csrc/lm_k_refine.hip
@@ -112,29 +112,92 @@
 #ifndef PRUNE_REFINE_PAIR
 #define PRUNE_REFINE_PAIR false
 #endif
-template <bool W4>
 __device__ __forceinline__ u32 rf_patch(const u8* __restrict__ lm, u32 se, u32 lane_off) {
-    if (W4) {
-        const u32x2 d = ld8a4(lm + ((se & ~3u) + lane_off));
-        return __builtin_amdgcn_alignbyte(d[1], d[0], se);
-    }
-    const u32 t = se + lane_off;
-    const u32x2 d = ld8a4(lm + (t & ~3u));
-    return __builtin_amdgcn_alignbyte(d[1], d[0], t);
+    const u32x2 d = ld8a4(lm + ((se & ~3u) + lane_off));
+    return __builtin_amdgcn_alignbyte(d[1], d[0], se);
+}
+__device__ __forceinline__ bool rf_locate(const LmRefineArgs& a, const LmRefFeat& ft, bool live, int bx, int by, u32& eff) {
+    const int col = (int)__umulhi((u32)ft.x << 1, a.tdiv) + bx, row = (int)__umulhi((u32)ft.y << 1, a.tdiv) + by;
+    const bool ok = live && col >= 0 && row >= 0 && col < a.g.W && row < a.g.H;
+    eff = ok ? (ft.off & 0x1FFFFFFFu) + lm_strip_off(a.g.H, row, col) : a.g.zero_off;
+    return ok;
+}
+__device__ __forceinline__ bool rf_wraps(const LmRefineArgs& a, const LmRefMeta& mt, int bx, int by) {
+    return bx + (int)(mt.qmax & 0xFFFFu) + 16 > a.g.W || by + (int)(mt.qmax >> 16) + 16 > a.g.H;
 }
 __device__ __forceinline__ void rf_lookup(const u8* __restrict__ tab, u32 v, u32 (&r)[4]) {
     r[0] = tab[v & 0xFFu]; r[1] = tab[(v >> 8) & 0xFFu]; r[2] = tab[(v >> 16) & 0xFFu]; r[3] = tab[v >> 24];
 }
-template <bool LAST, bool W4>
+template <bool LAST>
+__device__ __forceinline__ void refine_finish(const LmRefineArgs& a, LmDevHeader* hdr, u64* keys, LmCand* cand, u32 i, u32 ti, const u32 (&s)[4],
+                                              int bx, int by, int nfeat_total, int lane) {
+    const int T = a.g.T;
+    const int offset = T / 2 + (T % 2 - 1);
+    const u32 idx0 = (u32)lane * 4u;
+    const u32 k0 = (s[0] << 8) | (255u - idx0), k1 = (s[1] << 8) | (254u - idx0);
+    const u32 k2 = (s[2] << 8) | (253u - idx0), k3 = (s[3] << 8) | (252u - idx0);
+    const u32 k01 = k0 > k1 ? k0 : k1, k23 = k2 > k3 ? k2 : k3;
+    const u32 key = wave_max_u32(k01 > k23 ? k01 : k23);
+    const int best = (int)(key >> 8);
+    int best_r = -1, best_c = -1;
+    if (best > 0) { const int idx = 255 - (int)(key & 255u); best_r = idx >> 4; best_c = idx & 15; }
+    const int nx = (bx + best_c) * T + offset, ny = (by + best_r) * T + offset;
+    const float sim = __fdiv_rn(__fmul_rn((float)best, 100.f), (float)(4 * nfeat_total));
+    if (lane == 0) {
+        if (sim < a.threshold) {
+            if (a.stat) atomicAdd(&a.stat[5], 1ull);
+            cand[i].ti = LM_DROPPED;
+        } else if (LAST) {
+            emit_key(a, hdr, keys, ti, nx, ny, sim);
+        } else {
+            LmCand o; o.ti = ti; o.x = nx; o.y = ny; o.sim = sim;
+            cand[i] = o;
+        }
+    }
+}
+
+template <bool LAST>
+__device__ __forceinline__ void refine_one_wrap(const LmRefineArgs& a, u32 slot, u32 i, u32 ti, const LmRefMeta& mt, int bx, int by,
+                                                const u8 (*resp)[256], int lane) {
+    LmDevHeader* hdr = slot_ptr_s(a.hdr, a.aux_slot_stride, slot);
+    LmCand* cand = slot_ptr_s(a.cand, a.aux_slot_stride, slot);
+    u64* keys = slot_ptr_s(a.keys, a.aux_slot_stride, slot);
+    const u8* lm = a.lm + (size_t)slot * a.lm_slot_stride;
+    const int T = a.g.T, W = a.g.W, H = a.g.H;
+    const u32 ms = lm_strip_mem_bytes(W, H);
+    u32 s[4] = {0, 0, 0, 0};
+    for (int m = 0; m < a.M; ++m) {
+        const int cnt = (int)(m == 0 ? mt.count[0] : mt.count[1]);
+        const u32 fstart = m == 0 ? mt.start[0] : mt.start[1];
+        for (int f = 0; f < cnt; ++f) {
+            const LmRefFeat ft = a.feats[fstart + f];
+            const int qx = (int)__umulhi((u32)ft.x << 1, a.tdiv), qy = (int)__umulhi((u32)ft.y << 1, a.tdiv);
+            const int col = qx + bx, row = qy + by;
+            if (col < 0 || row < 0 || col >= W || row >= H) continue;
+            int g = (ft.y - qy * T) * T + (ft.x - qx * T), r = row + (lane >> 2), c = col + (lane & 3) * 4;
+            const u8* tab = resp[ft.off >> 29];
+#pragma unroll
+            for (int k = 0; k < 4; ++k, ++c) {
+                while (c >= W) { c -= W; ++r; }
+                while (r >= H) { r -= H; ++g; }
+                u32 v = 0;
+                if (g < T * T) v = lm[(size_t)m * a.g.mod_stride + (size_t)g * ms + lm_strip_off(H, r, c)];
+                s[k] += tab[v];
+            }
+        }
+    }
+    refine_finish<LAST>(a, hdr, keys, cand, i, ti, s, bx, by, mt.nfeat_total, lane);
+}
+
+template <bool LAST, bool WRAP>
 __device__ __forceinline__ void refine_one(const LmRefineArgs& a, u32 slot, u32 i, const u8 (*resp)[256], int lane) {
     LmDevHeader* hdr = slot_ptr_s(a.hdr, a.aux_slot_stride, slot);
     LmCand* cand = slot_ptr_s(a.cand, a.aux_slot_stride, slot);
     u64* keys = slot_ptr_s(a.keys, a.aux_slot_stride, slot);
     const u8* lm = a.lm + (size_t)slot * a.lm_slot_stride;
-    const int T = a.g.T, W = a.g.W;
+    const int T = a.g.T;
     const int border = 8 * T;
-    const int offset = T / 2 + (T % 2 - 1);
-    const u32 lane_off = (u32)((lane >> 2) * W + (lane & 3) * 4);
+    const u32 lane_off = (u32)((lane >> 2) * LM_STRIP_PITCH + (lane & 3) * 4);
     LmCand c = cand[i];
     u32 ti = (u32)__builtin_amdgcn_readfirstlane((int)c.ti);
     if (ti == LM_DROPPED) return;
@@ -145,8 +208,7 @@
     x = x > border ? x : border; y = y > border ? y : border;
     x = x < max_x ? x : max_x;  y = y < max_y ? y : max_y;
     int bx = x / T - 8, by = y / T - 8;
-    int off_x = bx * T, off_y = by * T;
-    const u32 shift = (u32)(by * W + bx);
+    if (WRAP && rf_wraps(a, mt, bx, by)) { refine_one_wrap<LAST>(a, slot, i, ti, mt, bx, by, resp, lane); return; }
     u32 s[4] = {0, 0, 0, 0};
     if (a.stat && lane == 0) atomicAdd(&a.stat[0], 1ull);
     int f_left = mt.nfeat_total;
@@ -158,14 +220,13 @@
         LmRefFeat ft;
         ft.off = 0; ft.x = 0; ft.y = 0;
         if (lane < cnt) ft = a.feats[fstart + lane];
-        int fx = ft.x + off_x, fy = ft.y + off_y;
-        bool ok = (lane < cnt) && fx >= 0 && fy >= 0 && fx < a.g.w && fy < a.g.h;
-        const u32 eff = ok ? (ft.off & 0x1FFFFFFFu) + shift : a.g.zero_off;
+        u32 eff;
+        (void)rf_locate(a, ft, lane < cnt, bx, by, eff);
         const u32 lab = ft.off >> 29;
         for (int f = 0; f < cnt; f += 8) {
             u32 v[8], q[8][4];
 #pragma unroll
-            for (int k = 0; k < 8; ++k) v[k] = rf_patch<W4>(lm, (u32)__builtin_amdgcn_readlane((int)eff, f + k), lane_off);
+            for (int k = 0; k < 8; ++k) v[k] = rf_patch(lm, (u32)__builtin_amdgcn_readlane((int)eff, f + k), lane_off);
 #pragma unroll
             for (int k = 0; k < 8; ++k) rf_lookup(resp[(u32)__builtin_amdgcn_readlane((int)lab, f + k)], v[k], q[k]);
 #pragma unroll
@@ -183,57 +244,33 @@
         if (a.stat && lane == 0) atomicAdd(&a.stat[4], 1ull);
         return;
     }
-    u32 idx0 = (u32)lane * 4u;
-    u32 k0 = (s[0] << 8) | (255u - idx0);
-    u32 k1 = (s[1] << 8) | (254u - idx0);
-    u32 k2 = (s[2] << 8) | (253u - idx0);
-    u32 k3 = (s[3] << 8) | (252u - idx0);
-    u32 k01 = k0 > k1 ? k0 : k1, k23 = k2 > k3 ? k2 : k3;
-    u32 key = wave_max_u32(k01 > k23 ? k01 : k23);
-    int best = (int)(key >> 8);
-    int best_r = -1, best_c = -1;
-    if (best > 0) { int idx = 255 - (int)(key & 255u); best_r = idx >> 4; best_c = idx & 15; }
-    int nx = (bx + best_c) * T + offset, ny = (by + best_r) * T + offset;
-    float sim = __fdiv_rn(__fmul_rn((float)best, 100.f), (float)(4 * mt.nfeat_total));
-    if (lane == 0) {
-        if (sim < a.threshold) {
-            if (a.stat) atomicAdd(&a.stat[5], 1ull);
-            cand[i].ti = LM_DROPPED;
-        } else if (LAST) {
-            emit_key(a, hdr, keys, ti, nx, ny, sim);
-        } else {
-            LmCand o; o.ti = ti; o.x = nx; o.y = ny; o.sim = sim;
-            cand[i] = o;
-        }
-    }
+    refine_finish<LAST>(a, hdr, keys, cand, i, ti, s, bx, by, mt.nfeat_total, lane);
 }
 
 #ifndef RP_BATCH
 #define RP_BATCH 8
 #endif
 static_assert(RP_BATCH % 2 == 0, "the responses are added two features at a time (v_add3_u32)");
-template <bool LAST, bool W4>
+template <bool LAST, bool WRAP>
 __device__ __forceinline__ void refine_pair(const LmRefineArgs& a, u32 slot, u32 i, const u8 (*resp)[256], int lane) {
     LmCand* cand = slot_ptr_s(a.cand, a.aux_slot_stride, slot);
     const u32 tiA = (u32)__builtin_amdgcn_readfirstlane((int)cand[i].ti);
     const u32 tiB = (u32)__builtin_amdgcn_readfirstlane((int)cand[i + 1].ti);
     if (tiA != tiB || tiA == LM_DROPPED) {
-        refine_one<LAST, W4>(a, slot, i, resp, lane);
-        refine_one<LAST, W4>(a, slot, i + 1, resp, lane);
+        refine_one<LAST, WRAP>(a, slot, i, resp, lane);
+        refine_one<LAST, WRAP>(a, slot, i + 1, resp, lane);
         return;
     }
     LmDevHeader* hdr = slot_ptr_s(a.hdr, a.aux_slot_stride, slot);
     u64* keys = slot_ptr_s(a.keys, a.aux_slot_stride, slot);
     const u8* lm = a.lm + (size_t)slot * a.lm_slot_stride;
-    const int T = a.g.T, W = a.g.W;
+    const int T = a.g.T;
     const int border = 8 * T;
-    const int offset = T / 2 + (T % 2 - 1);
-    const u32 lane_off = (u32)((lane >> 2) * W + (lane & 3) * 4);
+    const u32 lane_off = (u32)((lane >> 2) * LM_STRIP_PITCH + (lane & 3) * 4);
     const u32 ti = tiA;
     const LmRefMeta mt = a.meta[ti];
     const int max_x = a.g.w - mt.width - border, max_y = a.g.h - mt.height - border;
-    int bx[2], by[2], off_x[2], off_y[2];
-    u32 shift[2];
+    int bx[2], by[2];
 #pragma unroll
     for (int c = 0; c < 2; ++c) {
         const LmCand cd = cand[i + c];
@@ -242,8 +279,11 @@
         x = x > border ? x : border; y = y > border ? y : border;
         x = x < max_x ? x : max_x;  y = y < max_y ? y : max_y;
         bx[c] = x / T - 8; by[c] = y / T - 8;
-        off_x[c] = bx[c] * T; off_y[c] = by[c] * T;
-        shift[c] = (u32)(by[c] * W + bx[c]);
+    }
+    if (WRAP && (rf_wraps(a, mt, bx[0], by[0]) || rf_wraps(a, mt, bx[1], by[1]))) {
+        refine_one<LAST, WRAP>(a, slot, i, resp, lane);
+        refine_one<LAST, WRAP>(a, slot, i + 1, resp, lane);
+        return;
     }
     u32 s[2][4] = {{0, 0, 0, 0}, {0, 0, 0, 0}};
     if (a.stat && lane == 0) atomicAdd(&a.stat[1], 2ull);
@@ -260,14 +300,9 @@
         u32 eff[2];
         bool ok2[2];
 #pragma unroll
-        for (int c = 0; c < 2; ++c) {
-            const int fx = ft.x + off_x[c], fy = ft.y + off_y[c];
-            const bool ok = (lane < cnt) && fx >= 0 && fy >= 0 && fx < a.g.w && fy < a.g.h;
-            ok2[c] = ok;
-            eff[c] = ok ? (ft.off & 0x1FFFFFFFu) + shift[c] : a.g.zero_off;
-        }
+        for (int c = 0; c < 2; ++c) ok2[c] = rf_locate(a, ft, lane < cnt, bx[c], by[c], eff[c]);
         const u32 lab = ft.off >> 29;
-        const bool share = W4 && same_rows && __all(lane >= cnt || (ok2[0] && ok2[1]));
+        const bool share = same_rows && __all(lane >= cnt || (ok2[0] && ok2[1]));
         for (int f = 0; f < cnt; f += RP_BATCH) {
             u32 v[2][RP_BATCH], q[2][RP_BATCH][4];
             if (share) {
@@ -285,7 +320,7 @@
 #pragma unroll
             for (int k = 0; k < RP_BATCH; ++k)
 #pragma unroll
-                for (int c = 0; c < 2; ++c) v[c][k] = rf_patch<W4>(lm, (u32)__builtin_amdgcn_readlane((int)eff[c], f + k), lane_off);
+                for (int c = 0; c < 2; ++c) v[c][k] = rf_patch(lm, (u32)__builtin_amdgcn_readlane((int)eff[c], f + k), lane_off);
             }
 #pragma unroll
             for (int k = 0; k < RP_BATCH; ++k) {
@@ -311,40 +346,18 @@
                     if (a.stat && lane == 0) { atomicAdd(&a.stat[2], (unsigned long long)(out[0] + out[1])); if (out[0] && out[1]) atomicAdd(&a.stat[3], 1ull); }
                     if (out[0] && lane == 0) cand[i].ti = LM_DROPPED;
                     if (out[1] && lane == 0) cand[i + 1].ti = LM_DROPPED;
-                    if (!out[0]) refine_one<LAST, W4>(a, slot, i, resp, lane);
-                    if (!out[1]) refine_one<LAST, W4>(a, slot, i + 1, resp, lane);
+                    if (!out[0]) refine_one<LAST, WRAP>(a, slot, i, resp, lane);
+                    if (!out[1]) refine_one<LAST, WRAP>(a, slot, i + 1, resp, lane);
                     return;
                 }
             }
         }
     }
 #pragma unroll
-    for (int c = 0; c < 2; ++c) {
-        const u32 idx0 = (u32)lane * 4u;
-        const u32 k0 = (s[c][0] << 8) | (255u - idx0), k1 = (s[c][1] << 8) | (254u - idx0);
-        const u32 k2 = (s[c][2] << 8) | (253u - idx0), k3 = (s[c][3] << 8) | (252u - idx0);
-        const u32 k01 = k0 > k1 ? k0 : k1, k23 = k2 > k3 ? k2 : k3;
-        const u32 key = wave_max_u32(k01 > k23 ? k01 : k23);
-        const int best = (int)(key >> 8);
-        int best_r = -1, best_c = -1;
-        if (best > 0) { const int idx = 255 - (int)(key & 255u); best_r = idx >> 4; best_c = idx & 15; }
-        const int nx = (bx[c] + best_c) * T + offset, ny = (by[c] + best_r) * T + offset;
-        const float sim = __fdiv_rn(__fmul_rn((float)best, 100.f), (float)(4 * mt.nfeat_total));
-        if (lane == 0) {
-            if (sim < a.threshold) {
-                if (a.stat) atomicAdd(&a.stat[5], 1ull);
-                cand[i + c].ti = LM_DROPPED;
-            } else if (LAST) {
-                emit_key(a, hdr, keys, ti, nx, ny, sim);
-            } else {
-                LmCand o; o.ti = ti; o.x = nx; o.y = ny; o.sim = sim;
-                cand[i + c] = o;
-            }
-        }
-    }
-}
-
-template <bool LAST, bool W4>
+    for (int c = 0; c < 2; ++c) refine_finish<LAST>(a, hdr, keys, cand, i + c, ti, s[c], bx[c], by[c], mt.nfeat_total, lane);
+}
+
+template <bool LAST, bool WRAP>
 __global__ __launch_bounds__(256) void k_refine(LmRefineArgs a) {
     __shared__ u8 resp[8][256];
     const int lane = threadIdx.x & 63;
@@ -384,22 +397,22 @@
             while (idx + 1 < xlen && xpre[idx + 1] <= g) ++idx;
             const u32 i = g - xpre[idx] + xoff[idx];
             if (g + 1 < xpre[idx + 1]) {
-                refine_pair<LAST, W4>(a, xs[idx], i, resp, lane);
+                refine_pair<LAST, WRAP>(a, xs[idx], i, resp, lane);
             } else {
-                refine_one<LAST, W4>(a, xs[idx], i, resp, lane);
+                refine_one<LAST, WRAP>(a, xs[idx], i, resp, lane);
                 if (g + 1 < total) {
                     u32 idx2 = idx;
                     while (idx2 + 1 < xlen && xpre[idx2 + 1] <= g + 1) ++idx2;
-                    refine_one<LAST, W4>(a, xs[idx2], g + 1 - xpre[idx2] + xoff[idx2], resp, lane);
+                    refine_one<LAST, WRAP>(a, xs[idx2], g + 1 - xpre[idx2] + xoff[idx2], resp, lane);
                 }
             }
         }
     } else if (total <= nwaves) {
-        if (wave0 < total) refine_one<LAST, W4>(a, slot, wave0, resp, lane);
+        if (wave0 < total) refine_one<LAST, WRAP>(a, slot, wave0, resp, lane);
     } else {
         for (u32 i = 2u * wave0; i < total; i += 2u * nwaves) {
-            if (i + 1 < total) refine_pair<LAST, W4>(a, slot, i, resp, lane);
-            else refine_one<LAST, W4>(a, slot, i, resp, lane);
+            if (i + 1 < total) refine_pair<LAST, WRAP>(a, slot, i, resp, lane);
+            else refine_one<LAST, WRAP>(a, slot, i, resp, lane);
         }
     }
 }
@@ -641,9 +654,9 @@
     LmRefineArgs a = a_in;
     a.blocks_per_slot = 256; a.nslots = nslots;
     dim3 grid(a.plan ? (unsigned)(8 * a.blocks_per_slot) : (unsigned)(a.blocks_per_slot * nslots), 1, 1);
-    const bool w4 = (a.g.W & 3) == 0;
-    if (last) { if (w4) hipLaunchKernelGGL((k_refine<true, true>), grid, dim3(256), 0, s, a); else hipLaunchKernelGGL((k_refine<true, false>), grid, dim3(256), 0, s, a); }
-    else { if (w4) hipLaunchKernelGGL((k_refine<false, true>), grid, dim3(256), 0, s, a); else hipLaunchKernelGGL((k_refine<false, false>), grid, dim3(256), 0, s, a); }
+    a.tdiv = (u32)((1ull << 31) / (u32)a.g.T + 1u);
+    if (last) { if (a.wrap) hipLaunchKernelGGL((k_refine<true, true>), grid, dim3(256), 0, s, a); else hipLaunchKernelGGL((k_refine<true, false>), grid, dim3(256), 0, s, a); }
+    else { if (a.wrap) hipLaunchKernelGGL((k_refine<false, true>), grid, dim3(256), 0, s, a); else hipLaunchKernelGGL((k_refine<false, false>), grid, dim3(256), 0, s, a); }
 }
 
 void lmk_emit_unrefined(hipStream_t s, const LmRefineArgs& a, int nslots) {
diff --git a/line-mod-pipeline_amd/csrc/lm_kernels.h b/line-mod-pipeline_amd/csrc/lm_kernels.h
--- a/line-mod-pipeline_amd/csrc/lm_kernels.h
+++ b/line-mod-pipeline_amd/csrc/lm_kernels.h
@@ -126,6 +126,7 @@
     int M;
     const LmRefMeta* meta;
     const LmRefFeat* feats;
+    int wrap;
     const u32* sim_lut;
     LmDevHeader* hdr;
     LmCand* cand;
@@ -139,6 +140,7 @@
     const u32* plan;
     int plan_cap;
     int blocks_per_slot, nslots;
+    u32 tdiv;
     unsigned long long* stat;
 };
 void lmk_refine_plan(hipStream_t s, const LmRefineArgs& a, int nslots, u32* plan, int plan_cap);
```

Result: no change. 200,100, median of 6 (+0.8%).
